# apache/tez

Measured on NVIDIA H100. Metric: sorted KV GB/s (16B key / 64B val), higher is better.
Workload: dtype u8

## Files before the change

### tez_b200/csrc/radix_sort.cuh

```cuda
#pragma once
#include "common.cuh"

#ifndef TEZGPU_RADIX_THREADS32
#define TEZGPU_RADIX_THREADS32 384
#endif
#ifndef TEZGPU_RADIX_IPT32
#define TEZGPU_RADIX_IPT32 16
#endif
#ifndef TEZGPU_RADIX_MINB32
#define TEZGPU_RADIX_MINB32 (1024 / TEZGPU_RADIX_THREADS32)
#endif
#ifndef TEZGPU_RADIX_LOOKBACK
#define TEZGPU_RADIX_LOOKBACK 4
#endif
#ifndef TEZGPU_RANK_MODE
#define TEZGPU_RANK_MODE 2
#endif

namespace tezgpu {

constexpr int RADIX_BITS = 8;
constexpr int RADIX = 1 << RADIX_BITS;
constexpr uint32_t STATE_FLAG_LOCAL = 1u << 30;
constexpr uint32_t STATE_FLAG_INCL = 2u << 30;
constexpr uint32_t STATE_VALUE_MASK = (1u << 30) - 1;
constexpr uint32_t RADIX_MAX_N = (1u << 30) - 1;

template <typename KeyT>
__device__ __forceinline__ uint32_t radix_digit(KeyT k, int shift) {
  return (uint32_t)(k >> shift) & (RADIX - 1);
}

template <typename KeyT, int NPASS>
__global__ void __launch_bounds__(512) k_radix_hist(const KeyT *__restrict__ keys, uint32_t n, int begin_bit,
                                                    uint32_t *__restrict__ hist ) {
  __shared__ uint32_t s_hist[NPASS * RADIX];
  for (int i = threadIdx.x; i < NPASS * RADIX; i += blockDim.x) s_hist[i] = 0;
  __syncthreads();
  uint32_t stride = gridDim.x * blockDim.x;
  for (uint32_t i = blockIdx.x * blockDim.x + threadIdx.x; i < n; i += stride) {
    KeyT k = keys[i];
#pragma unroll
    for (int p = 0; p < NPASS; p++) atomicAdd(&s_hist[p * RADIX + radix_digit(k, begin_bit + p * RADIX_BITS)], 1u);
  }
  __syncthreads();
  for (int i = threadIdx.x; i < NPASS * RADIX; i += blockDim.x) {
    uint32_t c = s_hist[i];
    if (c) atomicAdd(&hist[i], c);
  }
}

__global__ void __launch_bounds__(RADIX) k_radix_scan_hist(uint32_t *__restrict__ hist, int npass, uint32_t n,
                                                          uint32_t *__restrict__ trivial) {
  __shared__ uint32_t s_warp[RADIX / 32];
  const int tid = threadIdx.x, lane = tid & 31, warp = tid >> 5;
  for (int p = 0; p < npass; p++) {
    uint32_t c = hist[p * RADIX + tid];
    uint32_t incl = c;
#pragma unroll
    for (int o = 1; o < 32; o <<= 1) {
      uint32_t t = __shfl_up_sync(0xffffffffu, incl, o);
      if (lane >= o) incl += t;
    }
    if (lane == 31) s_warp[warp] = incl;
    __syncthreads();
    uint32_t base = 0;
    for (int w = 0; w < warp; w++) base += s_warp[w];
    hist[p * RADIX + tid] = base + incl - c;
    uint32_t any = __syncthreads_or(c == n && n > 0);
    if (tid == 0 && trivial) trivial[p] = any ? 1u : 0u;
    __syncthreads();
  }
}

enum RadixIO : int { IO_SEP = 0, IO_SEP_IOTA = 1, IO_PAIR = 2 };

template <typename KeyT, int THREADS, int IPT>
struct OnesweepCfg {
  static constexpr int NWARPS = THREADS / 32;
  static constexpr int TILE = THREADS * IPT;
  static constexpr size_t SMEM = (size_t)TILE * (sizeof(KeyT) + sizeof(uint32_t)) + (size_t)NWARPS * RADIX * 4 +
                                 2 * RADIX * 4 + 64 + (TEZGPU_RANK_MODE == 2 ? (size_t)NWARPS * RADIX * 4 : 0);
};

template <typename KeyT, int THREADS, int IPT, int MINB, int IN, int OUT>
__global__ void __launch_bounds__(THREADS, MINB)
    k_onesweep_pass(const KeyT *__restrict__ keys_in, KeyT *__restrict__ keys_out, const uint32_t *__restrict__ vals_in,
                    uint32_t *__restrict__ vals_out, uint32_t n, int shift, const uint32_t *__restrict__ hist_base,
                    uint32_t *tile_state, uint32_t *tile_counter) {
  using Cfg = OnesweepCfg<KeyT, THREADS, IPT>;
  constexpr int NWARPS = Cfg::NWARPS;
  constexpr int TILE = Cfg::TILE;
  constexpr bool PAIRS = sizeof(KeyT) == 4;
  static_assert(THREADS >= RADIX, "one thread per digit for the look-back");
  static_assert(PAIRS || (IN != IO_PAIR && OUT != IO_PAIR), "pairs carry 32-bit keys");
  static_assert(OUT != IO_SEP_IOTA, "iota is an input layout");

  extern __shared__ __align__(16) uint8_t smem_raw[];
  uint2 *s_pair = reinterpret_cast<uint2 *>(smem_raw);
  KeyT *s_keys = reinterpret_cast<KeyT *>(smem_raw);
  uint32_t *s_vals = reinterpret_cast<uint32_t *>(smem_raw + (size_t)TILE * sizeof(KeyT));
  uint32_t *s_wcnt = s_vals + TILE;
  uint32_t *s_dstart = s_wcnt + NWARPS * RADIX;
  uint32_t *s_goff = s_dstart + RADIX;
  uint32_t *s_misc = s_goff + RADIX;
#if TEZGPU_RANK_MODE == 2
  uint32_t *s_wmask = s_misc + 16;
#endif

  const int tid = threadIdx.x, lane = tid & 31, warp = tid >> 5;

#ifdef TEZGPU_TICKET_ATOMIC
  if (tid == 0) s_misc[0] = atomicAdd(tile_counter, 1u);
#else
  if (tid == 0) s_misc[0] = blockIdx.x;
#endif
  for (int i = tid; i < NWARPS * RADIX; i += THREADS) s_wcnt[i] = 0;
#if TEZGPU_RANK_MODE == 2
  for (int i = tid; i < NWARPS * RADIX; i += THREADS) s_wmask[i] = 0;
#endif
  __syncthreads();
  const uint32_t tile = s_misc[0];
  const uint32_t tile_base = tile * (uint32_t)TILE;
  const uint32_t tile_n = min((uint32_t)TILE, n - tile_base);
  const uint32_t warp_base = (uint32_t)warp * 32u * IPT;

  KeyT key[IPT];
  uint32_t val[IN == IO_SEP_IOTA ? 1 : IPT];
  uint32_t rnk[IPT];
#pragma unroll
  for (int j = 0; j < IPT; j++) {
    const uint32_t li = warp_base + j * 32 + lane;
    const bool valid = li < tile_n;
    if constexpr (IN == IO_PAIR) {
      uint2 p = make_uint2(~0u, 0u);
      if (valid) p = reinterpret_cast<const uint2 *>(keys_in)[tile_base + li];
      key[j] = p.x;
      val[j] = p.y;
    } else {
      key[j] = valid ? keys_in[tile_base + li] : ~(KeyT)0;
      if constexpr (IN == IO_SEP) val[j] = valid ? vals_in[tile_base + li] : 0u;
    }
  }
  uint32_t *wc = s_wcnt + warp * RADIX;
  const uint32_t lt = lanemask_lt();
#pragma unroll
  for (int j = 0; j < IPT; j++) {
    const uint32_t d = radix_digit(key[j], shift);
    uint32_t peers;
#if TEZGPU_RANK_MODE == 0
    peers = __match_any_sync(0xffffffffu, d);
#elif TEZGPU_RANK_MODE == 2
    {
      uint32_t *wm = s_wmask + warp * RADIX;
      atomicOr(&wm[d], 1u << lane);
      __syncwarp();
      peers = wm[d];
      __syncwarp();
      atomicAnd(&wm[d], ~(1u << lane));
    }
#else
    peers = 0xffffffffu;
#pragma unroll
    for (int b = 0; b < RADIX_BITS; b++) {
      const bool bit = (d >> b) & 1u;
      const uint32_t bm = __ballot_sync(0xffffffffu, bit);
      peers &= bit ? bm : ~bm;
    }
#endif
    uint32_t pre = 0;
    if ((peers & lt) == 0) pre = atomicAdd(&wc[d], (uint32_t)__popc(peers));
    pre = __shfl_sync(0xffffffffu, pre, __ffs(peers) - 1);
    rnk[j] = pre + __popc(peers & lt);
  }
  __syncthreads();

  uint32_t count = 0;
  if (tid < RADIX) {
    uint32_t run = 0;
#pragma unroll
    for (int w = 0; w < NWARPS; w++) {
      uint32_t c = s_wcnt[w * RADIX + tid];
      s_wcnt[w * RADIX + tid] = run;
      run += c;
    }
    count = run;
    st_relaxed_gpu_u32(&tile_state[(size_t)tile * RADIX + tid], (tile == 0 ? STATE_FLAG_INCL : STATE_FLAG_LOCAL) | count);
    uint32_t incl = count;
#pragma unroll
    for (int o = 1; o < 32; o <<= 1) {
      uint32_t t = __shfl_up_sync(0xffffffffu, incl, o);
      if (lane >= o) incl += t;
    }
    if (lane == 31) s_misc[1 + warp] = incl;
    s_dstart[tid] = incl - count;
  }
  __syncthreads();
  if (tid < RADIX) {
    uint32_t base = 0;
    for (int w = 0; w < warp; w++) base += s_misc[1 + w];
    s_dstart[tid] += base;
  }
  __syncthreads();

#pragma unroll
  for (int j = 0; j < IPT; j++) {
    const uint32_t d = radix_digit(key[j], shift);
    const uint32_t slot = s_dstart[d] + wc[d] + rnk[j];
    uint32_t v;
    if constexpr (IN == IO_SEP_IOTA) v = tile_base + warp_base + j * 32 + lane;
    else v = val[j];
    if constexpr (PAIRS) {
      s_pair[slot] = make_uint2((uint32_t)key[j], v);
    } else {
      s_keys[slot] = key[j];
      s_vals[slot] = v;
    }
  }

  if (tid < RADIX) {
    uint32_t excl = 0;
    if (tile > 0) {
      constexpr int LOOKBACK = TEZGPU_RADIX_LOOKBACK;
      int64_t t = (int64_t)tile - 1;
      bool done = false;
      while (!done) {
        uint32_t st[LOOKBACK];
#ifdef TEZGPU_RADIX_DEBUG
        if (tid == 0) atomicAdd(tile_counter + 7, 1u);
#endif
#pragma unroll
        for (int b = 0; b < LOOKBACK; b++)
          st[b] = (t - b >= 0) ? ld_relaxed_gpu_u32(&tile_state[(size_t)(t - b) * RADIX + tid]) : STATE_FLAG_INCL;
#pragma unroll
        for (int b = 0; b < LOOKBACK; b++) {
          if (done) break;
          uint32_t flag = st[b] & ~STATE_VALUE_MASK;
          if (flag == 0) break;
          excl += st[b] & STATE_VALUE_MASK;
          t--;
          if (flag == STATE_FLAG_INCL) done = true;
        }
      }
      st_relaxed_gpu_u32(&tile_state[(size_t)tile * RADIX + tid], STATE_FLAG_INCL | (excl + count));
    }
    s_goff[tid] = hist_base[tid] + excl - s_dstart[tid];
  }
  __syncthreads();

#pragma unroll
  for (int k = 0; k < IPT; k++) {
    const uint32_t slot = (uint32_t)tid + k * THREADS;
    if (slot < tile_n) {
      KeyT kk;
      uint32_t v;
      if constexpr (PAIRS) {
        const uint2 p = s_pair[slot];
        kk = p.x;
        v = p.y;
      } else {
        kk = s_keys[slot];
        v = s_vals[slot];
      }
      const uint32_t dest = s_goff[radix_digit(kk, shift)] + slot;
      if constexpr (OUT == IO_PAIR) {
        reinterpret_cast<uint2 *>(keys_out)[dest] = make_uint2((uint32_t)kk, v);
      } else {
        keys_out[dest] = kk;
        vals_out[dest] = v;
      }
    }
  }
}

struct RadixWorkspace {
  uint32_t *hist = nullptr;
  uint32_t *trivial = nullptr;
  uint32_t *tile_state = nullptr;
  uint32_t *tile_counter = nullptr;
  size_t tile_state_words = 0;
};

template <typename KeyT>
struct RadixTuning {
  static constexpr int THREADS = sizeof(KeyT) == 4 ? TEZGPU_RADIX_THREADS32 : 512;
  static constexpr int IPT = sizeof(KeyT) == 4 ? TEZGPU_RADIX_IPT32 : 10;
  static constexpr int MINB = sizeof(KeyT) == 4 ? TEZGPU_RADIX_MINB32 : 2;
};

template <typename KeyT>
static inline uint32_t radix_num_tiles(uint32_t n) {
  using T = RadixTuning<KeyT>;
  return (uint32_t)div_up(n, (uint64_t)T::THREADS * T::IPT);
}
template <typename KeyT>
static inline size_t radix_tile_state_words(uint32_t n, int npass) {
  return (size_t)radix_num_tiles<KeyT>(n) * RADIX * (size_t)npass;
}

template <typename KeyT, int IN, int OUT>
static void radix_launch_pass(cudaStream_t st, uint32_t ntiles, const KeyT *kin, KeyT *kout, const uint32_t *vin,
                              uint32_t *vout, uint32_t n, int shift, const uint32_t *hist, uint32_t *state,
                              uint32_t *counter) {
  using T = RadixTuning<KeyT>;
  using Cfg = OnesweepCfg<KeyT, T::THREADS, T::IPT>;
  auto kern = k_onesweep_pass<KeyT, T::THREADS, T::IPT, T::MINB, IN, OUT>;
  static bool attr_set = false;
  if (!attr_set) {
    TG_CUDA(cudaFuncSetAttribute(kern, cudaFuncAttributeMaxDynamicSharedMemorySize, (int)Cfg::SMEM));
    attr_set = true;
  }
  kern<<<ntiles, T::THREADS, Cfg::SMEM, st>>>(kin, kout, vin, vout, n, shift, hist, state, counter);
  TG_CUDA(cudaGetLastError());
}

template <typename KeyT>
static uint32_t radix_prepare(cudaStream_t st, const RadixWorkspace &ws, uint32_t n, int npass) {
  const uint32_t ntiles = radix_num_tiles<KeyT>(n);
  TG_CHECK((size_t)ntiles * RADIX * (size_t)npass <= ws.tile_state_words, -1, "radix workspace too small");
  TG_CUDA(cudaMemsetAsync(ws.tile_state, 0, (size_t)ntiles * RADIX * (size_t)npass * 4, st));
  TG_CUDA(cudaMemsetAsync(ws.tile_counter, 0, 8 * 4, st));
  return ntiles;
}


static int radix_sort_pairs(cudaStream_t st, const RadixWorkspace &ws, uint32_t *blk_a, uint32_t *blk_b, uint32_t n,
                            int begin_bit, int npass, uint32_t pass_mask, int *launches) {
  const int total = __builtin_popcount(pass_mask & ((1u << npass) - 1));
  TG_CHECK(total >= 1, -1, "radix sort without a pass");
  const uint32_t ntiles = radix_prepare<uint32_t>(st, ws, n, npass);
  int done = 0;
  for (int p = 0; p < npass; p++) {
    if (!((pass_mask >> p) & 1u)) continue;
    uint32_t *in = (done & 1) ? blk_b : blk_a, *out = (done & 1) ? blk_a : blk_b;
    const bool first = done == 0, last = done + 1 == total;
    const int shift = begin_bit + p * RADIX_BITS;
    const uint32_t *hist = ws.hist + p * RADIX;
    uint32_t *state = ws.tile_state + (size_t)p * ntiles * RADIX, *counter = ws.tile_counter + p;
    if (first && last)
      radix_launch_pass<uint32_t, IO_SEP_IOTA, IO_SEP>(st, ntiles, in, out, nullptr, out + n, n, shift, hist, state, counter);
    else if (first)
      radix_launch_pass<uint32_t, IO_SEP_IOTA, IO_PAIR>(st, ntiles, in, out, nullptr, nullptr, n, shift, hist, state, counter);
    else if (last)
      radix_launch_pass<uint32_t, IO_PAIR, IO_SEP>(st, ntiles, in, out, nullptr, out + n, n, shift, hist, state, counter);
    else
      radix_launch_pass<uint32_t, IO_PAIR, IO_PAIR>(st, ntiles, in, out, nullptr, nullptr, n, shift, hist, state, counter);
    if (launches) (*launches)++;
    done++;
  }
  return done;
}

template <typename KeyT>
static int radix_sort_passes(cudaStream_t st, const RadixWorkspace &ws, KeyT *keys_a, KeyT *keys_b, uint32_t *vals_a,
                             uint32_t *vals_b, uint32_t n, int begin_bit, int npass, uint32_t pass_mask, int *launches) {
  static_assert(sizeof(KeyT) == 8, "32-bit keys are sorted as pairs (radix_sort_pairs)");
  const uint32_t ntiles = radix_prepare<KeyT>(st, ws, n, npass);
  int done = 0;
  for (int p = 0; p < npass; p++) {
    if (!((pass_mask >> p) & 1u)) continue;
    KeyT *kin = (done & 1) ? keys_b : keys_a, *kout = (done & 1) ? keys_a : keys_b;
    uint32_t *vin = (done & 1) ? vals_b : vals_a, *vout = (done & 1) ? vals_a : vals_b;
    radix_launch_pass<KeyT, IO_SEP, IO_SEP>(st, ntiles, kin, kout, vin, vout, n, begin_bit + p * RADIX_BITS,
                                            ws.hist + p * RADIX, ws.tile_state + (size_t)p * ntiles * RADIX,
                                            ws.tile_counter + p);
    if (launches) (*launches)++;
    done++;
  }
  return done;
}

}
```

### tez_b200/csrc/scan.cuh

```cuda
#pragma once
#include "common.cuh"

namespace tezgpu {

constexpr int SCAN_THREADS = 256;
constexpr int SCAN_IPT = 8;
constexpr int SCAN_TILE = SCAN_THREADS * SCAN_IPT;

__device__ __forceinline__ uint64_t block_exclusive_scan_u64(uint64_t v, uint64_t *s_warp ,
                                                             uint64_t *total) {
  const int lane = threadIdx.x & 31, warp = threadIdx.x >> 5;
  uint64_t incl = v;
#pragma unroll
  for (int o = 1; o < 32; o <<= 1) {
    uint64_t t = __shfl_up_sync(0xffffffffu, incl, o);
    if (lane >= o) incl += t;
  }
  if (lane == 31) s_warp[warp] = incl;
  __syncthreads();
  uint64_t base = 0, tot = 0;
#pragma unroll
  for (int w = 0; w < SCAN_THREADS / 32; w++) {
    uint64_t x = s_warp[w];
    if (w < warp) base += x;
    tot += x;
  }
  __syncthreads();
  if (total) *total = tot;
  return base + incl - v;
}

__global__ void __launch_bounds__(1024) k_scan_block_sums(uint64_t *blk, uint32_t nblk) {
  __shared__ uint64_t s_warp[32];
  __shared__ uint64_t s_carry;
  const int lane = threadIdx.x & 31, warp = threadIdx.x >> 5;
  if (threadIdx.x == 0) s_carry = 0;
  __syncthreads();
  for (uint32_t base = 0; base < nblk; base += 1024) {
    uint32_t i = base + threadIdx.x;
    uint64_t v = i < nblk ? blk[i] : 0, incl = v;
#pragma unroll
    for (int o = 1; o < 32; o <<= 1) {
      uint64_t t = __shfl_up_sync(0xffffffffu, incl, o);
      if (lane >= o) incl += t;
    }
    if (lane == 31) s_warp[warp] = incl;
    __syncthreads();
    uint64_t wbase = 0, tot = 0;
    for (int w = 0; w < 32; w++) {
      uint64_t x = s_warp[w];
      if (w < warp) wbase += x;
      tot += x;
    }
    uint64_t carry = s_carry;
    if (i < nblk) blk[i] = carry + wbase + incl - v;
    __syncthreads();
    if (threadIdx.x == 0) s_carry = carry + tot;
    __syncthreads();
  }
  if (threadIdx.x == 0) blk[nblk] = s_carry;
}

__global__ void __launch_bounds__(SCAN_THREADS) k_sum_u32_blocks(const uint32_t *__restrict__ in, uint32_t n,
                                                                 uint64_t *__restrict__ blk) {
  __shared__ uint64_t s_warp[SCAN_THREADS / 32];
  uint32_t base = blockIdx.x * SCAN_TILE;
  uint64_t s = 0;
#pragma unroll
  for (int k = 0; k < SCAN_IPT; k++) {
    uint32_t i = base + k * SCAN_THREADS + threadIdx.x;
    if (i < n) s += in[i];
  }
  uint64_t tot;
  block_exclusive_scan_u64(s, s_warp, &tot);
  if (threadIdx.x == 0) blk[blockIdx.x] = tot;
}

__global__ void __launch_bounds__(SCAN_THREADS) k_scan_u32_apply(const uint32_t *__restrict__ in, uint32_t n,
                                                                 const uint64_t *__restrict__ blk,
                                                                 uint64_t *__restrict__ out) {
  __shared__ uint64_t s_warp[SCAN_THREADS / 32];
  uint32_t base = blockIdx.x * SCAN_TILE + threadIdx.x * SCAN_IPT;
  uint32_t v[SCAN_IPT];
  uint64_t s = 0;
#pragma unroll
  for (int k = 0; k < SCAN_IPT; k++) {
    uint32_t i = base + k;
    v[k] = i < n ? in[i] : 0;
    s += v[k];
  }
  uint64_t ex = block_exclusive_scan_u64(s, s_warp, nullptr) + blk[blockIdx.x];
#pragma unroll
  for (int k = 0; k < SCAN_IPT; k++) {
    uint32_t i = base + k;
    if (i < n) out[i] = ex;
    ex += v[k];
  }
  if (blockIdx.x == gridDim.x - 1 && threadIdx.x == SCAN_THREADS - 1) out[n] = blk[gridDim.x];
}

}
```

### tez_b200/csrc/sorter.cuh

```cuda
#pragma once
#include <stdlib.h>
#include <string.h>

#include <vector>

#include "../../include/tezgpu.h"
#include "device_util.h"
#include "combine.cuh"
#include "deflate.cuh"
#include "emit_pipe_u.cuh"
#include "sorter_kernels.cuh"

namespace tezgpu {

__global__ void k_store_to_host(uint32_t *__restrict__ dst0, const uint32_t *__restrict__ src0, uint32_t n0, uint32_t *__restrict__ dst1,
                                const uint32_t *__restrict__ src1, uint32_t n1, uint32_t *__restrict__ dst2,
                                const uint32_t *__restrict__ src2, uint32_t n2) {
  for (uint32_t i = threadIdx.x; i < n0; i += blockDim.x) dst0[i] = src0[i];
  for (uint32_t i = threadIdx.x; i < n1; i += blockDim.x) dst1[i] = src1[i];
  for (uint32_t i = threadIdx.x; i < n2; i += blockDim.x) dst2[i] = src2[i];
  __threadfence_system();
}
static inline void store_to_host(cudaStream_t st, void *d0, const void *s0, size_t b0, void *d1 = nullptr, const void *s1 = nullptr,
                                 size_t b1 = 0, void *d2 = nullptr, const void *s2 = nullptr, size_t b2 = 0) {
  k_store_to_host<<<1, 256, 0, st>>>((uint32_t *)d0, (const uint32_t *)s0, (uint32_t)(b0 / 4), (uint32_t *)d1, (const uint32_t *)s1,
                                     (uint32_t)(b1 / 4), (uint32_t *)d2, (const uint32_t *)s2, (uint32_t)(b2 / 4));
}


static inline int partition_bits(int P) {
  int b = 0;
  while ((1ll << b) < (long long)P) b++;
  return b;
}

struct DeviceConstants {
  CrcTables *d_crc = nullptr;
  static DeviceConstants &get(int device) {
    static DeviceConstants inst[64];
    DeviceConstants &d = inst[device & 63];
    if (!d.d_crc) {
      CrcTables *h = new CrcTables();
      crc_build_tables(*h, EMIT_CRC_STRIDE_WORDS);
      TG_CUDA(cudaMalloc((void **)&d.d_crc, sizeof(CrcTables)));
      TG_CUDA(cudaMemcpy(d.d_crc, h, sizeof(CrcTables), cudaMemcpyHostToDevice));
      delete h;
    }
    return d;
  }
};

struct FramingMismatch {};

enum class FixedEmitKernel {
  Pipe,
  Fast,
  PipeUnaligned,
  FastUnaligned,
  General,
};
struct FixedEmitPlan {
  FixedEmitKernel kernel;
  uint32_t recs_per_tile;
};

static inline FixedEmitPlan plan_fixed_emit(const Records &rec, uint32_t rec_size) {
  const uint32_t stride = rec.klen + rec.vlen, cpr = stride / 16;
  const uint32_t cap = std::max<uint32_t>(1, std::min<uint32_t>(EMIT_MAX_RECS, (FE_IMG_BYTES - 32) / rec_size));
  if (stride < 16 || stride % 16) return {FixedEmitKernel::General, cap};
  if (!rec.key_off && !rec.use_runs && ((uintptr_t)rec.kv & 15u) == 0) {
    const uint32_t m = emit4_max_recs(rec_size);
    if (emit4_fits(m, cpr, rec_size)) return {FixedEmitKernel::Pipe, std::min(cap, m)};
    return {FixedEmitKernel::Fast, cap};
  }
  const uint32_t m = emit4u_max_recs(cpr);
  if (m == 0) return {FixedEmitKernel::FastUnaligned, cap};
  const uint32_t top = std::min(cap, m);
  uint32_t best = top;
  double best_eff = 0;
  for (uint32_t r = top; r >= top - top / 10; r--) {
    const uint64_t chunks = ((uint64_t)r * rec_size + 15 + 4 + 2 + 15) / 16;
    const uint64_t rounds = (chunks + FE_THREADS - 1) / FE_THREADS;
    const double eff = (double)r / (double)rounds;
    if (eff > best_eff) { best_eff = eff; best = r; }
  }
  return {FixedEmitKernel::PipeUnaligned, best};
}

class SortPipeline {
 public:
  tezgpu_conf conf;
  int pbits;
  cudaStream_t stream = nullptr;
  EventTimer timer;
  int num_sms = 132;

  DeviceBuffer sortA, sortB, same, blk, small, tile_state, sizes, rec_off;
  DeviceBuffer t_pos[2], t_gid[2], t_lidx[2], t_key64[2], t_val[2], t_state, t_ghead, t_gneq, sym_sets, sym_tab, rep_flags;
  DeviceBuffer seg_start, tile_start, part_start, d_index, seg_crc, tile_desc, tile_crc, tie_state;
  PinnedBuffer h_small;

  explicit SortPipeline(const tezgpu_conf &c) : conf(c) {
    TG_CHECK(c.num_partitions >= 1, TEZGPU_E_INVALID, "num_partitions must be >= 1");
    TG_CHECK(c.comparator >= TEZGPU_CMP_BYTES && c.comparator <= TEZGPU_CMP_LONG, TEZGPU_E_UNSUPPORTED,
             "comparator outside the device-supported set (BYTES, TEXT, BYTESWRITABLE, INT, LONG)");
    TG_CHECK(c.partitioner == TEZGPU_PART_GIVEN || c.partitioner == TEZGPU_PART_HASH, TEZGPU_E_UNSUPPORTED,
             "partitioner outside the device-supported set (GIVEN, HASH)");
    int ndev = 0;
    cudaError_t e = cudaGetDeviceCount(&ndev);
    if (e != cudaSuccess || ndev == 0) {
      cudaGetLastError();
      throw Error(TEZGPU_E_CUDA, "no CUDA device available (libtezgpu has no CPU fallback)");
    }
    TG_CHECK(c.device >= 0 && c.device < ndev, TEZGPU_E_INVALID, "bad device ordinal");
    TG_CUDA(cudaSetDevice(c.device));
    TG_CUDA(cudaStreamCreateWithFlags(&stream, cudaStreamNonBlocking));
    TG_CUDA(cudaDeviceGetAttribute(&num_sms, cudaDevAttrMultiProcessorCount, c.device));
    {
      const char *g = getenv("TEZGPU_L2_FETCH");
      int gran = g ? atoi(g) : 32;
      if (gran > 0 && cudaDeviceSetLimit(cudaLimitMaxL2FetchGranularity, (size_t)gran) != cudaSuccess) cudaGetLastError();
    }
    pbits = partition_bits(c.num_partitions);
    TG_CHECK(pbits <= 31, TEZGPU_E_INVALID, "too many partitions");
    h_small.ensure(4096);
    small.ensure(16384);
    DeviceConstants::get(c.device);
  }
  ~SortPipeline() {
    if (stream) cudaStreamDestroy(stream);
  }

  static uint64_t output_bound(uint64_t n, uint64_t kv_bytes, int P) { return kv_bytes + 12 * n + 10ull * P + 64; }

  uint32_t *d_hist() { return small.as<uint32_t>(); }
  uint32_t *d_trivial() { return small.as<uint32_t>() + 2048; }
  uint32_t *d_tile_counter() { return small.as<uint32_t>() + 2056; }
  int *d_error() { return reinterpret_cast<int *>(small.as<uint32_t>() + 2064); }
  uint32_t *d_large() { return small.as<uint32_t>() + 2065; }
  uint32_t *d_m() { return small.as<uint32_t>() + 2072; }
  unsigned long long *d_ties() { return reinterpret_cast<unsigned long long *>(small.as<uint32_t>() + 2074); }
  uint32_t *d_ticket() { return small.as<uint32_t>() + 2073; }
  unsigned long long *d_dups() { return reinterpret_cast<unsigned long long *>(small.as<uint32_t>() + 2066); }
  uint64_t *d_totals() { return reinterpret_cast<uint64_t *>(small.as<uint32_t>() + 2068); }

  struct SortState {
    Records rec;
    uint32_t *K = nullptr;
    uint32_t *order = nullptr;
    uint64_t dup_count = 0, tie_records = 0;
    int launches = 0;
    bool have_bounds = false, spec_layout = false;
    uint64_t spec_file_bytes = 0, spec_tiles = 0;
    const uint8_t *same = nullptr;
  } state;
  int merge_check_same = 1;
  bool merge_inputs_plain = false;
  int combiner = TEZGPU_COMBINE_NONE;
  DeviceBuffer c_head, c_gid, c_sums, c_hpos, c_K, c_order, c_same, c_kv, c_koff, c_klen, c_vlen, c_bad;
  PinnedBuffer c_host;
  EventTimer c_timer;

  EmitParams make_emit_params(const Records &rec, const uint32_t *order, int rle, bool merge_mode, uint8_t *d_out) {
    EmitParams e;
    memset(&e, 0, sizeof(e));
    e.rec = rec;
    e.order = order;
    e.same = state.same ? state.same : same.as<uint8_t>();
    e.part_start = part_start.as<uint32_t>();
    e.seg_start = seg_start.as<uint64_t>();
    e.tile_start = tile_start.as<uint32_t>();
    e.out = d_out;
    e.seg_crc = seg_crc.as<uint32_t>();
    e.crc = DeviceConstants::get(conf.device).d_crc;
    e.rle = rle;
    e.send_empty = conf.send_empty_partition_details;
    e.unordered = conf.sorter_impl == TEZGPU_SORTER_UNORDERED;
    e.merge_mode = merge_mode ? 1 : 0;
    e.check_same = merge_check_same;
    e.P = conf.num_partitions;
    return e;
  }
  FixedEmitKernel set_fixed_layout(EmitParams &e, const Records &rec) {
    int h = 0;
    for (int b = 0; b < vint_size_u32(rec.klen); b++) e.fixed_hdr[h++] = vint_byte_u32(rec.klen, b);
    for (int b = 0; b < vint_size_u32(rec.vlen); b++) e.fixed_hdr[h++] = vint_byte_u32(rec.vlen, b);
    e.fixed_hdr_len = h;
    e.rec_size = h + rec.klen + rec.vlen;
    const FixedEmitPlan plan = plan_fixed_emit(rec, e.rec_size);
    e.recs_per_tile = plan.recs_per_tile;
    e.rec_off = nullptr;
    return plan.kernel;
  }

  void run(Records rec, uint8_t *d_out, uint64_t out_cap, uint64_t *out_len, int64_t *index, tezgpu_stats *stats) {
    const uint64_t raw_bound = output_bound(rec.n, rec.fixed ? (uint64_t)rec.n * (rec.klen + rec.vlen) : rec.kv_bytes, conf.num_partitions);
    sort_phase(rec);
    int rle;
    if (conf.rle_policy == TEZGPU_RLE_ON) rle = 1;
    else if (conf.rle_policy == TEZGPU_RLE_OFF) rle = 0;
    else rle = (conf.sorter_impl == 1) ? 0 : ((double)state.dup_count > 0.1 * (double)rec.n);
    if (conf.sorter_impl == TEZGPU_SORTER_UNORDERED) rle = 0;
    emit_out(rle, false, raw_bound, d_out, out_cap, out_len, index, stats);
  }

  int codec = TEZGPU_CODEC_NONE;
  DeviceBuffer z_img, z_slots, z_csize, z_cadler, z_coff, z_segs, z_descs, z_pstart, z_tc, z_crc;
  PinnedBuffer z_host;
  EventTimer z_timer;
  static uint64_t codec_bound(int codec, uint64_t raw_bound, int P);
  void compress_image(const int64_t *raw_index, uint8_t *d_out, uint64_t out_cap, uint64_t *out_len, int64_t *index, tezgpu_stats *stats);

  void emit_out(int rle, bool merge_mode, uint64_t raw_bound, uint8_t *d_out, uint64_t out_cap, uint64_t *out_len, int64_t *index,
                tezgpu_stats *stats) {
    if (!codec) {
      if (combiner) emit_combined(rle, d_out, out_cap, out_len, index, stats);
      else emit_phase(rle, merge_mode, d_out, out_cap, out_len, index, stats);
      return;
    }
    const int P = conf.num_partitions;
    z_img.ensure(raw_bound + 64);
    std::vector<int64_t> raw_index((size_t)P * 3, 0);
    uint64_t raw_len = 0;
    tezgpu_stats st;
    memset(&st, 0, sizeof(st));
    if (combiner) emit_combined(rle, z_img.as<uint8_t>(), z_img.cap, &raw_len, raw_index.data(), &st);
    else emit_phase(rle, merge_mode, z_img.as<uint8_t>(), z_img.cap, &raw_len, raw_index.data(), &st);
    compress_image(raw_index.data(), d_out, out_cap, out_len, index, &st);
    if (stats) *stats = st;
  }

  void sort_phase(Records rec) {
    TG_CUDA(cudaSetDevice(conf.device));
    const uint32_t n = rec.n;
    const int P = conf.num_partitions;
    TG_CHECK(n <= RADIX_MAX_N, TEZGPU_E_INVALID, "more than 2^30-1 records in one sort");
    rec.cmp = conf.comparator;
    rec.hash_partition = conf.partitioner == TEZGPU_PART_HASH;
    rec.num_partitions = P;
    rec.pbits = pbits;
    const bool unordered = conf.sorter_impl == TEZGPU_SORTER_UNORDERED;
    rec.unordered = unordered ? 1 : 0;
    TG_CHECK(rec.hash_partition || rec.partition || rec.use_runs || n == 0 || P == 1, TEZGPU_E_INVALID, "partition ids required (partitioner=GIVEN)");
    int launches = 0;
    state.have_bounds = state.spec_layout = false;
    state.same = nullptr;
    timer.reset();
    timer.mark(stream);

    const size_t n4 = (size_t)(n ? n : 1) * 4;
    sortA.ensure(2 * n4); sortB.ensure(2 * n4);
    same.ensure(n ? n : 1);
    const uint32_t nblk = (uint32_t)div_up(n ? n : 1, SCAN_TILE);
    blk.ensure(((size_t)nblk + 2) * 8);
    part_start.ensure(((size_t)P + 1) * 4);
    seg_start.ensure(((size_t)P + 1) * 8);
    tile_start.ensure(((size_t)P + 1) * 4);
    d_index.ensure((size_t)P * 24);
    seg_crc.ensure((size_t)P * 4);
    h_small.ensure(4096 + (size_t)P * 24);

    TG_CUDA(cudaMemsetAsync(small.p, 0, 16384, stream));
    TG_CUDA(cudaMemsetAsync(seg_crc.p, 0, (size_t)P * 4, stream));

    uint64_t dup_count = 0;
    uint64_t tie_records = 0;
    uint32_t *K = sortA.as<uint32_t>();
    uint32_t *order = sortA.as<uint32_t>() + n;

    uint32_t sym_npos = 0;
    if (n && !rec.fixed && !unordered && !(getenv("TEZGPU_NO_SYM") && atoi(getenv("TEZGPU_NO_SYM")))) {
      sym_sets.ensure(SYM_MAX_POS * 8 * 4);
      sym_tab.ensure(sizeof(SymTable));
      TG_CUDA(cudaMemsetAsync(sym_sets.p, 0, SYM_MAX_POS * 8 * 4, stream));
      k_symbols<<<(int)std::min<uint64_t>(div_up(n, 256), (uint64_t)num_sms * 8), 256, 0, stream>>>(rec, sym_sets.as<uint32_t>());
      launches++;
      uint32_t hs[SYM_MAX_POS * 8];
      TG_CUDA(cudaMemcpyAsync(hs, sym_sets.p, sizeof(hs), cudaMemcpyDeviceToHost, stream));
      TG_CUDA(cudaStreamSynchronize(stream));
      SymTable *t = new SymTable();
      const uint32_t np = sym_table_build(hs, pbits, t);
      if (sym_table_pays(np, pbits)) {
        TG_CUDA(cudaMemcpyAsync(sym_tab.p, t, sizeof(SymTable), cudaMemcpyHostToDevice, stream));
        TG_CUDA(cudaStreamSynchronize(stream));
        rec.sym = sym_tab.as<SymTable>();
        sym_npos = np;
      }
      delete t;
    }
    if (n) {
      TG_CUDA(cudaMemsetAsync(same.p, 0, n, stream));
      const bool fast16 = rec.fixed && !rec.key_off && !rec.use_runs && rec.klen == 16 && ((rec.klen + rec.vlen) % 16 == 0) && rec.cmp == CMP_BYTES &&
                          (((uintptr_t)rec.kv & 15u) == 0);
      int sgrid = (int)std::min<uint64_t>(div_up(n, 256), (uint64_t)num_sms * 16);
      if (fast16) k_stage<true><<<sgrid, 256, 0, stream>>>(rec, K, d_hist(), d_error());
      else k_stage<false><<<sgrid, 256, 0, stream>>>(rec, K, d_hist(), d_error());
      TG_CUDA(cudaGetLastError());
      k_radix_scan_hist<<<1, RADIX, 0, stream>>>(d_hist(), 4, n, d_trivial());
      TG_CUDA(cudaGetLastError());
      launches += 2;
      timer.mark(stream);

      RadixWorkspace ws;
      ws.hist = d_hist();
      ws.trivial = d_trivial();
      ws.tile_counter = d_tile_counter();
      ws.tile_state_words = radix_tile_state_words<uint32_t>(n, 4);
      tile_state.ensure(ws.tile_state_words * 4);
      ws.tile_state = tile_state.as<uint32_t>();
      uint32_t pass_mask = 0xF;
      if (unordered) {
        pass_mask = 0;
        for (int q = 0; q < 4; q++) if (8 * q + 8 > 32 - pbits) pass_mask |= 1u << q;
        if (!pass_mask) pass_mask = 1;
      }
      int done = radix_sort_pairs(stream, ws, sortA.as<uint32_t>(), sortB.as<uint32_t>(), n, 0, 4, pass_mask, &launches);
      if (done & 1) { K = sortB.as<uint32_t>(); order = sortB.as<uint32_t>() + n; }
      if (unordered) {
        k_flip_order<<<(uint32_t)div_up(n, 256), 256, 0, stream>>>(order, n);
        launches++;
      }
      timer.mark(stream);

      const uint32_t depth0 = rec.sym ? sym_npos : (uint32_t)((32 - pbits) / 8);
      int per_sm_tf = 0;
      TG_CUDA(cudaOccupancyMaxActiveBlocksPerMultiprocessor(&per_sm_tf, k_tie_fix, TIEFIX_THREADS, 0));
      if (!unordered)
        k_tie_fix<<<(uint32_t)std::min<uint64_t>(div_up(n, TIEFIX_TILE), (uint64_t)num_sms * std::max(per_sm_tf, 1)), TIEFIX_THREADS, 0, stream>>>(
            rec, K, order, n, depth0, same.as<uint8_t>(), d_dups(), d_large(), d_ties());
      const uint32_t *d_m_ptr = reinterpret_cast<const uint32_t *>(d_ties());
      k_part_bounds<<<(uint32_t)div_up((uint64_t)P + 1, 256), 256, 0, stream>>>(K, n, P, pbits, part_start.as<uint32_t>());
      launches += 2;
      state.have_bounds = true;
      state.spec_layout = false;
      if (rec.fixed) {
        EmitParams e = make_emit_params(rec, order, 0, false, nullptr);
        set_fixed_layout(e, rec);
        k_layout<<<1, 1024, 0, stream>>>(e, seg_start.as<uint64_t>(), tile_start.as<uint32_t>(), d_index.as<int64_t>(), d_totals());
        launches++;
        state.spec_layout = true;
      }
      TG_CUDA(cudaGetLastError());
      uint32_t *hw = h_small.as<uint32_t>();
      store_to_host(stream, hw, small.as<uint32_t>() + 2064, 32, hw + 8, d_m_ptr, 4, h_small.as<uint8_t>() + 4096, d_index.p,
                    state.spec_layout ? (size_t)P * 24 : 0);
      TG_CUDA(cudaGetLastError());
      TG_CUDA(cudaStreamSynchronize(stream));
      TG_CHECK(!(hw[0] & 1u), TEZGPU_E_INVALID, "Illegal partition (outside [0, numPartitions))");
      if (hw[0] & 2u) throw FramingMismatch();
      uint32_t m = hw[8];
      tie_records = m;
      memcpy(&dup_count, hw + 2, 8);
      memcpy(&state.spec_file_bytes, hw + 4, 8);
      memcpy(&state.spec_tiles, hw + 6, 8);
      uint64_t *hs = h_small.as<uint64_t>() + 16;
      if (hw[1]) {
        k_tie_count<<<nblk, SCAN_THREADS, 0, stream>>>(K, n, blk.as<uint64_t>());
        k_scan_block_sums<<<1, 1024, 0, stream>>>(blk.as<uint64_t>(), nblk);
        TG_CUDA(cudaMemcpyAsync(&hs[0], blk.as<uint64_t>() + nblk, 8, cudaMemcpyDeviceToHost, stream));
        TG_CUDA(cudaStreamSynchronize(stream));
        m = (uint32_t)hs[0];
        tie_records = m;
        for (int s2 = 0; s2 < 2; s2++) { t_pos[s2].ensure((size_t)m * 4); t_gid[s2].ensure((size_t)m * 4); t_lidx[s2].ensure((size_t)m * 4); }
        k_tie_compact<<<nblk, SCAN_THREADS, 0, stream>>>(K, order, n, blk.as<uint64_t>(), t_pos[0].as<uint32_t>(),
                                                         t_gid[0].as<uint32_t>(), t_lidx[0].as<uint32_t>());
        launches += 3;
        const uint32_t ngroups = (uint32_t)(hs[0] >> 32);
        int cur = 0;
        {
          t_ghead.ensure(((size_t)ngroups + 2) * 4);
          t_gneq.ensure((size_t)ngroups + 1);
          TG_CUDA(cudaMemsetAsync(t_gneq.p, 0, (size_t)ngroups + 1, stream));
          const uint32_t mgrid = (uint32_t)div_up(m, 256), mblk0 = (uint32_t)div_up(m, SCAN_TILE);
          k_group_heads<<<mgrid, 256, 0, stream>>>(t_gid[0].as<uint32_t>(), m, t_ghead.as<uint32_t>());
          k_group_equal<<<mgrid, 256, 0, stream>>>(rec, t_gid[0].as<uint32_t>(), t_lidx[0].as<uint32_t>(), t_ghead.as<uint32_t>(), m, depth0,
                                                 TIE_SMALL_MAX, t_gneq.as<uint8_t>());
          blk.ensure(((size_t)std::max(mblk0, nblk) + 2) * 8);
          k_group_mark<<<mblk0, SCAN_THREADS, 0, stream>>>(t_pos[0].as<uint32_t>(), t_gid[0].as<uint32_t>(), t_ghead.as<uint32_t>(),
                                                          t_gneq.as<uint8_t>(), m, TIE_SMALL_MAX, same.as<uint8_t>(), d_dups(), blk.as<uint64_t>());
          k_scan_block_sums<<<1, 1024, 0, stream>>>(blk.as<uint64_t>(), mblk0);
          launches += 4;
          TG_CUDA(cudaGetLastError());
          TG_CUDA(cudaMemcpyAsync(&hs[0], blk.as<uint64_t>() + mblk0, 8, cudaMemcpyDeviceToHost, stream));
          TG_CUDA(cudaStreamSynchronize(stream));
          const uint32_t m2 = (uint32_t)hs[0];
          if (m2) {
            k_group_compact<<<mblk0, SCAN_THREADS, 0, stream>>>(t_pos[0].as<uint32_t>(), t_gid[0].as<uint32_t>(), t_lidx[0].as<uint32_t>(),
                                                               t_ghead.as<uint32_t>(), t_gneq.as<uint8_t>(), m, TIE_SMALL_MAX, blk.as<uint64_t>(),
                                                               t_pos[1].as<uint32_t>(), t_gid[1].as<uint32_t>(), t_lidx[1].as<uint32_t>());
            launches++;
            TG_CUDA(cudaGetLastError());
            cur = 1;
          }
          m = m2;
        }
        uint32_t depth = depth0;
        while (m) {
          t_key64[0].ensure((size_t)m * 8); t_key64[1].ensure((size_t)m * 8); t_val[0].ensure((size_t)m * 4);
          const uint32_t mblk = (uint32_t)div_up(m, SCAN_TILE);
          k_ref_build_keys<<<(uint32_t)div_up(m, 256), 256, 0, stream>>>(rec, t_gid[cur].as<uint32_t>(), t_lidx[cur].as<uint32_t>(), m,
                                                                    depth, t_key64[0].as<uint64_t>());
          TG_CUDA(cudaMemsetAsync(d_hist(), 0, 8 * RADIX * 4, stream));
          k_radix_hist<uint64_t, 8><<<(int)std::min<uint64_t>(div_up(m, 512 * 8), (uint64_t)num_sms * 4), 512, 0, stream>>>(t_key64[0].as<uint64_t>(), m, 0, d_hist());
          k_radix_scan_hist<<<1, RADIX, 0, stream>>>(d_hist(), 8, m, d_trivial());
          launches += 3;
          TG_CUDA(cudaGetLastError());
          uint32_t *ht = h_small.as<uint32_t>() + 64;
          TG_CUDA(cudaMemcpyAsync(ht, d_trivial(), 8 * 4, cudaMemcpyDeviceToHost, stream));
          TG_CUDA(cudaStreamSynchronize(stream));
          uint32_t mask = 0;
          for (int q = 0; q < 8; q++) if (!ht[q]) mask |= 1u << q;
          RadixWorkspace w2 = ws;
          w2.tile_state_words = radix_tile_state_words<uint64_t>(m, 8);
          t_state.ensure(w2.tile_state_words * 4);
          w2.tile_state = t_state.as<uint32_t>();
          int d2 = radix_sort_passes<uint64_t>(stream, w2, t_key64[0].as<uint64_t>(), t_key64[1].as<uint64_t>(), t_lidx[cur].as<uint32_t>(),
                                               t_val[0].as<uint32_t>(), m, 0, 8, mask, &launches);
          const uint64_t *Ks = (d2 & 1) ? t_key64[1].as<uint64_t>() : t_key64[0].as<uint64_t>();
          const uint32_t *Ls = (d2 & 1) ? t_val[0].as<uint32_t>() : t_lidx[cur].as<uint32_t>();
          k_ref_apply_count<<<mblk, SCAN_THREADS, 0, stream>>>(Ks, Ls, t_pos[cur].as<uint32_t>(), m, order, same.as<uint8_t>(), d_dups(),
                                                              blk.as<uint64_t>());
          k_scan_block_sums<<<1, 1024, 0, stream>>>(blk.as<uint64_t>(), mblk);
          launches += 2;
          TG_CUDA(cudaMemcpyAsync(&hs[0], blk.as<uint64_t>() + mblk, 8, cudaMemcpyDeviceToHost, stream));
          TG_CUDA(cudaStreamSynchronize(stream));
          uint32_t m2 = (uint32_t)hs[0];
          if (m2) {
            k_ref_compact<<<mblk, SCAN_THREADS, 0, stream>>>(Ks, Ls, t_pos[cur].as<uint32_t>(), m, blk.as<uint64_t>(),
                                                            t_pos[cur ^ 1].as<uint32_t>(), t_gid[cur ^ 1].as<uint32_t>(),
                                                            t_lidx[cur ^ 1].as<uint32_t>());
            launches++;
            TG_CUDA(cudaGetLastError());
          }
          cur ^= 1;
          m = m2;
          depth += 3;
        }
        TG_CUDA(cudaMemcpyAsync(&hs[0], d_dups(), 8, cudaMemcpyDeviceToHost, stream));
        TG_CUDA(cudaStreamSynchronize(stream));
        dup_count = hs[0];
      }
    }
    timer.mark(stream);
    state.rec = rec;
    state.K = K;
    state.order = order;
    state.dup_count = dup_count;
    state.tie_records = tie_records;
    state.launches = launches;
  }

  void emit_phase(int rle, bool merge_mode, uint8_t *d_out, uint64_t out_cap, uint64_t *out_len, int64_t *index,
                  tezgpu_stats *stats) {
    TG_CUDA(cudaSetDevice(conf.device));
    TG_CHECK(((uintptr_t)d_out & 15u) == 0, TEZGPU_E_INVALID, "output buffer must be 16-byte aligned");
    const Records rec = state.rec;
    const uint32_t n = rec.n;
    const int P = conf.num_partitions;
    uint32_t *K = state.K, *order = state.order;
    const uint64_t dup_count = state.dup_count, tie_records = state.tie_records;
    int launches = state.launches;
    const CrcTables *d_crc = DeviceConstants::get(conf.device).d_crc;
    const size_t n4 = (size_t)(n ? n : 1) * 4;
    const uint32_t nblk = (uint32_t)div_up(n ? n : 1, SCAN_TILE);
    TG_CUDA(cudaMemsetAsync(seg_crc.p, 0, (size_t)P * 4, stream));
    if (timer.n > (n ? 4 : 2)) timer.n = n ? 4 : 2;

    EmitParams e = make_emit_params(rec, order, rle, merge_mode, d_out);
    if (!state.have_bounds) {
      k_part_bounds<<<(uint32_t)div_up((uint64_t)P + 1, 256), 256, 0, stream>>>(K, n, P, pbits, part_start.as<uint32_t>());
      launches++;
    }
    const bool no_repeats = !rle && (!merge_mode || (!merge_check_same && merge_inputs_plain));
    const bool fixed_emit = rec.fixed && (dup_count == 0 || no_repeats);
    uint64_t bound = output_bound(n, rec.fixed ? (uint64_t)n * (rec.klen + rec.vlen) : rec.kv_bytes, P);
    uint64_t *hs = h_small.as<uint64_t>();
    const FixedEmitKernel kernel = fixed_emit ? set_fixed_layout(e, rec) : FixedEmitKernel::General;
    if (fixed_emit && state.spec_layout) {
      hs[0] = state.spec_file_bytes;
      hs[1] = state.spec_tiles;
    } else {
      if (!fixed_emit) {
        uint64_t avg = n ? (rec.fixed ? (uint64_t)(rec.klen + rec.vlen) : rec.kv_bytes / n) + 4 : 16;
        e.recs_per_tile = (uint32_t)std::max<uint64_t>(1, std::min<uint64_t>(EMIT_MAX_RECS, (EMIT_IMG_BYTES - 32) / avg));
        sizes.ensure(n4);
        rec_off.ensure(((size_t)n + 2) * 8);
        if (n) {
          rep_flags.ensure(n);
          k_emit_repeat_flags<<<(uint32_t)div_up(n, 256), 256, 0, stream>>>(e, K, rep_flags.as<uint8_t>());
          launches++;
          e.rep = rep_flags.as<uint8_t>();
          k_emit_sizes<<<(uint32_t)div_up(n, 256), 256, 0, stream>>>(e, K, sizes.as<uint32_t>());
          k_sum_u32_blocks<<<nblk, SCAN_THREADS, 0, stream>>>(sizes.as<uint32_t>(), n, blk.as<uint64_t>());
          k_scan_block_sums<<<1, 1024, 0, stream>>>(blk.as<uint64_t>(), nblk);
          k_scan_u32_apply<<<nblk, SCAN_THREADS, 0, stream>>>(sizes.as<uint32_t>(), n, blk.as<uint64_t>(), rec_off.as<uint64_t>());
          launches += 4;
          TG_CUDA(cudaGetLastError());
        } else {
          TG_CUDA(cudaMemsetAsync(rec_off.p, 0, 16, stream));
        }
        e.rec_off = rec_off.as<uint64_t>();
      }
      k_layout<<<1, 1024, 0, stream>>>(e, seg_start.as<uint64_t>(), tile_start.as<uint32_t>(), d_index.as<int64_t>(), d_totals());
      launches++;
      TG_CUDA(cudaGetLastError());
      store_to_host(stream, &hs[0], d_totals(), 16, h_small.as<uint8_t>() + 4096, d_index.p, (size_t)P * 24);
      TG_CUDA(cudaGetLastError());
      TG_CUDA(cudaStreamSynchronize(stream));
      state.spec_layout = false;
    }
    const uint64_t file_bytes = hs[0];
    const uint64_t tiles = hs[1];
    TG_CHECK(file_bytes <= bound, TEZGPU_E_INVALID, "internal: output exceeds bound");
    TG_CHECK(file_bytes <= out_cap, TEZGPU_E_NOMEM, "output buffer too small for file.out");
    const bool source_oriented = fixed_emit && kernel != FixedEmitKernel::General;
    const uint32_t stride = rec.klen + rec.vlen;
    FastEmitParams fp;
    if (tiles && source_oriented) {
      tile_desc.ensure((size_t)tiles * sizeof(TileDesc));
      k_build_tiles<<<(uint32_t)div_up(tiles, 256), 256, 0, stream>>>(e, tile_desc.as<TileDesc>());
      launches++;
      fp.e = e;
      tile_crc.ensure((size_t)tiles * sizeof(TileCrc));
      fp.tile_crc = tile_crc.as<TileCrc>();
      fp.tiles = tile_desc.as<TileDesc>();
      fp.ntiles = (uint32_t)tiles;
      fp.cpr = stride / 16;
      fp.cpr_magic = fp.cpr == 1 ? 0u : (uint32_t)((1ull << 32) / fp.cpr) + 1u;
      fp.stride = stride;
    }
    timer.mark(stream);
    if (tiles) {
      auto persistent_grid = [&](auto kern, int threads, size_t smem) {
        int per_sm = 0;
        TG_CUDA(cudaOccupancyMaxActiveBlocksPerMultiprocessor(&per_sm, kern, threads, smem));
        return (uint32_t)std::min<uint64_t>(tiles, (uint64_t)num_sms * (per_sm > 0 ? per_sm : 1));
      };
      if (!fixed_emit) {
        k_emit<false><<<persistent_grid(k_emit<false>, EMIT_THREADS, 0), EMIT_THREADS, 0, stream>>>(e);
      } else {
        switch (kernel) {
          case FixedEmitKernel::Pipe: {
            static bool attr = false;
            if (!attr) {
              TG_CUDA(cudaFuncSetAttribute(k_emit_fast4<FE4_UNROLL>, cudaFuncAttributeMaxDynamicSharedMemorySize, (int)Emit4Smem::TOTAL));
              attr = true;
            }
            const uint32_t grid = (uint32_t)std::min<uint64_t>(div_up(tiles, FE4_GROUPS), (uint64_t)num_sms);
            k_emit_fast4<FE4_UNROLL><<<grid, FE_THREADS * FE4_GROUPS, Emit4Smem::TOTAL, stream>>>(fp);
            break;
          }
          case FixedEmitKernel::Fast:
            k_emit_fast<5, true><<<persistent_grid(k_emit_fast<5, true>, FE_THREADS, 0), FE_THREADS, 0, stream>>>(fp);
            break;
          case FixedEmitKernel::PipeUnaligned: {
            static bool attr = false;
            if (!attr) {
              TG_CUDA(cudaFuncSetAttribute(k_emit_fast4u<FE4U_UNROLL>, cudaFuncAttributeMaxDynamicSharedMemorySize, (int)Emit4uSmem::TOTAL));
              attr = true;
            }
            const uint32_t grid = persistent_grid(k_emit_fast4u<FE4U_UNROLL>, FE_THREADS, Emit4uSmem::TOTAL);
            k_emit_fast4u<FE4U_UNROLL><<<grid, FE_THREADS, Emit4uSmem::TOTAL, stream>>>(fp);
            break;
          }
          case FixedEmitKernel::FastUnaligned:
            k_emit_fast<5, false><<<persistent_grid(k_emit_fast<5, false>, FE_THREADS, 0), FE_THREADS, 0, stream>>>(fp);
            break;
          case FixedEmitKernel::General:
            k_emit<true><<<persistent_grid(k_emit<true>, EMIT_THREADS, 0), EMIT_THREADS, 0, stream>>>(e);
            break;
        }
      }
      if (source_oriented) {
        k_crc_combine<<<(uint32_t)div_up(tiles, 256), 256, 0, stream>>>(fp.tile_crc, (uint32_t)tiles, d_crc, seg_crc.as<uint32_t>());
        launches++;
      }
      launches++;
      TG_CUDA(cudaGetLastError());
    }
    timer.mark(stream);
    k_finalize_segments<<<(uint32_t)div_up(P, 256), 256, 0, stream>>>(e);
    launches++;
    TG_CUDA(cudaGetLastError());
    timer.mark(stream);
    TG_CUDA(cudaStreamSynchronize(stream));

    if (out_len) *out_len = file_bytes;
    const int64_t *hidx = reinterpret_cast<const int64_t *>(h_small.as<uint8_t>() + 4096);
    if (index) memcpy(index, hidx, (size_t)P * 24);
    if (stats) {
      memset(stats, 0, sizeof(*stats));
      stats->output_records = n;
      int64_t raw = 0;
      for (int p = 0; p < P; p++) raw += hidx[3 * p + 1];
      stats->output_bytes_with_overhead = raw;
      stats->output_bytes_physical = (int64_t)file_bytes;
      stats->file_out_bytes = (int64_t)file_bytes;
      stats->spilled_records = n;
      stats->num_spills = 1;
      stats->rle_used = rle;
      stats->adjacent_equal_keys = (int64_t)dup_count;
      stats->tie_records = (int64_t)tie_records;
      const int b = n ? 3 : 1;
      stats->ms_stage = n ? timer.ms(0, 1) : 0;
      stats->ms_sort = n ? timer.ms(1, 2) : 0;
      stats->ms_ties = n ? timer.ms(2, 3) : 0;
      stats->ms_emit = timer.ms(b, b + 3);
      stats->ms_emit_kernel = timer.ms(b + 1, b + 2);
      stats->ms_total = timer.ms(0, b + 3);
      stats->kernel_launches = launches;
    }
  }

  bool combine_phase() {
    const Records rec = state.rec;
    const uint32_t n = rec.n, W = combine_width(combiner);
    TG_CHECK(W, TEZGPU_E_INVALID, "unknown combiner");
    const char *name = combiner == TEZGPU_COMBINE_SUM_INT ? "IntSumReducer needs 4-byte IntWritable values"
                                                          : "LongSumReducer needs 8-byte LongWritable values";
    if (n == 0) return false;
    c_bad.ensure(16);
    c_host.ensure(64);
    uint32_t *bad = c_bad.as<uint32_t>();
    TG_CUDA(cudaMemsetAsync(bad, 0xFF, 4, stream));
    int launches = 0;
    if (state.dup_count == 0) {
      if (rec.fixed) {
        TG_CHECK(rec.vlen == W, TEZGPU_E_INVALID, "combiner: record 0 has a " + std::to_string(rec.vlen) + "-byte value (" + name + ")");
        return false;
      }
      k_combine_check_width<<<(uint32_t)std::min<uint64_t>(div_up(n, 256), (uint64_t)num_sms * 16), 256, 0, stream>>>(rec, W, bad);
      TG_CUDA(cudaGetLastError());
      state.launches += 1;
      uint32_t *h = c_host.as<uint32_t>();
      TG_CUDA(cudaMemcpyAsync(h, bad, 4, cudaMemcpyDeviceToHost, stream));
      TG_CUDA(cudaStreamSynchronize(stream));
      TG_CHECK(h[0] == 0xFFFFFFFFu, TEZGPU_E_INVALID, "combiner: record " + std::to_string(h[0]) + " has a value of the wrong width (" + name + ")");
      return false;
    }
    const uint32_t nblk = (uint32_t)div_up(n, SCAN_TILE);
    c_head.ensure((size_t)n * 4);
    c_gid.ensure(((size_t)n + 1) * 8);
    blk.ensure(((size_t)nblk + 2) * 8);
    k_combine_heads<<<(uint32_t)div_up(n, 256), 256, 0, stream>>>(same.as<uint8_t>(), n, c_head.as<uint32_t>());
    k_sum_u32_blocks<<<nblk, SCAN_THREADS, 0, stream>>>(c_head.as<uint32_t>(), n, blk.as<uint64_t>());
    k_scan_block_sums<<<1, 1024, 0, stream>>>(blk.as<uint64_t>(), nblk);
    k_scan_u32_apply<<<nblk, SCAN_THREADS, 0, stream>>>(c_head.as<uint32_t>(), n, blk.as<uint64_t>(), c_gid.as<uint64_t>());
    launches += 4;
    c_sums.ensure((size_t)n * 8);
    c_hpos.ensure((size_t)n * 4);
    c_K.ensure((size_t)n * 4);
    TG_CUDA(cudaMemsetAsync(c_sums.p, 0, (size_t)n * 8, stream));
    const uint32_t sgrid = (uint32_t)div_up(div_up(n, 32 * CMB_ROWS) * 32, CMB_THREADS);
    if (W == 4)
      k_combine_sum<4><<<sgrid, CMB_THREADS, 0, stream>>>(rec, state.order, state.K, c_gid.as<uint64_t>(), n, c_sums.as<unsigned long long>(),
                                                          c_hpos.as<uint32_t>(), c_K.as<uint32_t>(), bad);
    else
      k_combine_sum<8><<<sgrid, CMB_THREADS, 0, stream>>>(rec, state.order, state.K, c_gid.as<uint64_t>(), n, c_sums.as<unsigned long long>(),
                                                          c_hpos.as<uint32_t>(), c_K.as<uint32_t>(), bad);
    launches++;
    TG_CUDA(cudaGetLastError());
    uint32_t *h = c_host.as<uint32_t>();
    TG_CUDA(cudaMemcpyAsync(h, bad, 4, cudaMemcpyDeviceToHost, stream));
    TG_CUDA(cudaMemcpyAsync(h + 2, c_gid.as<uint64_t>() + n, 8, cudaMemcpyDeviceToHost, stream));
    TG_CUDA(cudaStreamSynchronize(stream));
    TG_CHECK(h[0] == 0xFFFFFFFFu, TEZGPU_E_INVALID, "combiner: record " + std::to_string(h[0]) + " has a value of the wrong width (" + name + ")");
    uint64_t m64;
    memcpy(&m64, h + 2, 8);
    const uint32_t m = (uint32_t)m64;
    c_order.ensure((size_t)m * 4);
    c_same.ensure(m);
    TG_CUDA(cudaMemsetAsync(c_same.p, 0, m, stream));
    Records out;
    memset(&out, 0, sizeof(out));
    out.n = m;
    out.cmp = rec.cmp;
    out.hash_partition = rec.hash_partition;
    out.num_partitions = rec.num_partitions;
    out.pbits = rec.pbits;
    const uint64_t *off = nullptr;
    uint64_t bytes;
    if (rec.fixed) {
      bytes = (uint64_t)m * (rec.klen + W);
      out.fixed = 1;
      out.klen = rec.klen;
      out.vlen = W;
    } else {
      const uint32_t mblk = (uint32_t)div_up(m, SCAN_TILE);
      k_combine_sizes<<<(uint32_t)div_up(m, 256), 256, 0, stream>>>(rec, state.order, c_hpos.as<uint32_t>(), m, W, c_head.as<uint32_t>());
      k_sum_u32_blocks<<<mblk, SCAN_THREADS, 0, stream>>>(c_head.as<uint32_t>(), m, blk.as<uint64_t>());
      k_scan_block_sums<<<1, 1024, 0, stream>>>(blk.as<uint64_t>(), mblk);
      k_scan_u32_apply<<<mblk, SCAN_THREADS, 0, stream>>>(c_head.as<uint32_t>(), m, blk.as<uint64_t>(), c_gid.as<uint64_t>());
      launches += 4;
      TG_CUDA(cudaGetLastError());
      TG_CUDA(cudaMemcpyAsync(h + 4, c_gid.as<uint64_t>() + m, 8, cudaMemcpyDeviceToHost, stream));
      TG_CUDA(cudaStreamSynchronize(stream));
      memcpy(&bytes, h + 4, 8);
      off = c_gid.as<uint64_t>();
      c_koff.ensure((size_t)m * 8);
      c_klen.ensure((size_t)m * 4);
      c_vlen.ensure((size_t)m * 4);
      out.key_off = c_koff.as<uint64_t>();
      out.key_len = c_klen.as<uint32_t>();
      out.val_len = c_vlen.as<uint32_t>();
    }
    c_kv.ensure(align_up(bytes, 16) + 32);
    out.kv = c_kv.as<uint8_t>();
    out.kv_bytes = rec.fixed ? bytes : align_up(bytes, 16);
    const bool narrow = rec.fixed && rec.klen <= 64;
    const uint32_t lanes = narrow ? 1 : 32;
    const uint32_t wgrid = (uint32_t)div_up((uint64_t)m * lanes, 256);
    auto write = [&](auto kern) {
      kern<<<wgrid, 256, 0, stream>>>(rec, state.order, c_hpos.as<uint32_t>(), c_sums.as<unsigned long long>(), m, off, c_kv.as<uint8_t>(),
                                      c_order.as<uint32_t>(), c_koff.as<uint64_t>(), c_klen.as<uint32_t>(), c_vlen.as<uint32_t>());
    };
    if (W == 4) narrow ? write(k_combine_write<4, 1>) : write(k_combine_write<4, 32>);
    else narrow ? write(k_combine_write<8, 1>) : write(k_combine_write<8, 32>);
    launches++;
    TG_CUDA(cudaGetLastError());
    state.rec = out;
    state.K = c_K.as<uint32_t>();
    state.order = c_order.as<uint32_t>();
    state.same = c_same.as<uint8_t>();
    state.dup_count = 0;
    state.have_bounds = state.spec_layout = false;
    state.launches += launches;
    return true;
  }

  void emit_combined(int rle, uint8_t *d_out, uint64_t out_cap, uint64_t *out_len, int64_t *index, tezgpu_stats *stats) {
    const SortState saved = state;
    c_timer.reset();
    c_timer.mark(stream);
    bool replaced = false;
    try {
      replaced = combine_phase();
      c_timer.mark(stream);
      emit_phase(rle, false, d_out, out_cap, out_len, index, stats);
    } catch (...) {
      restore_after_combine(saved, replaced);
      throw;
    }
    const uint64_t written = state.rec.n;
    restore_after_combine(saved, replaced);
    if (stats) {
      const float ms_combine = c_timer.ms(0, 1);
      stats->output_records = (int64_t)saved.rec.n;
      stats->spilled_records = (int64_t)written;
      stats->adjacent_equal_keys = (int64_t)saved.dup_count;
      stats->ms_emit = std::max(0.f, stats->ms_emit - ms_combine);
    }
  }
  void restore_after_combine(const SortState &saved, bool replaced) {
    if (!replaced) return;
    const int launches = state.launches;
    state = saved;
    state.launches = launches;
    state.have_bounds = state.spec_layout = false;
  }
};

}
```

### tez_b200/csrc/sorter_kernels.cuh

```cuda
#pragma once
#include "common.cuh"
#include "crc32.cuh"
#include "radix_sort.cuh"
#include "scan.cuh"

namespace tezgpu {

struct RunTable {
  const uint64_t *seg_off;
  const uint32_t *rec_base;
  const uint32_t *seg_part;
  const uint32_t *part_seg0;
  uint32_t nseg;
  uint32_t rec_size;
  uint32_t hdr_len;
  uint64_t hdr_bytes;
};

__device__ __forceinline__ uint32_t run_of(const RunTable &t, uint32_t i) {
  uint32_t lo = 0, hi = t.nseg;
  while (hi - lo > 1) {
    const uint32_t mid = (lo + hi) >> 1;
    if (__ldg(t.rec_base + mid) <= i) lo = mid; else hi = mid;
  }
  return lo;
}
__device__ __forceinline__ uint32_t run_of_in_partition(const RunTable &t, uint32_t p, uint32_t i) {
  uint32_t seg = __ldg(t.part_seg0 + p);
  const uint32_t end = __ldg(t.part_seg0 + p + 1);
  while (seg + 1 < end && i >= __ldg(t.rec_base + seg + 1)) seg++;
  return seg;
}
__device__ __forceinline__ uint64_t run_record_off(const RunTable &t, uint32_t i, uint32_t &seg) {
  seg = run_of(t, i);
  return __ldg(t.seg_off + seg) + (uint64_t)(i - __ldg(t.rec_base + seg)) * t.rec_size;
}
__device__ __forceinline__ uint64_t run_record_off_p(const RunTable &t, uint32_t p, uint32_t i) {
  const uint32_t seg = run_of_in_partition(t, p, i);
  return __ldg(t.seg_off + seg) + (uint64_t)(i - __ldg(t.rec_base + seg)) * t.rec_size;
}

constexpr int SYM_MAX_POS = 16;
struct SymTable {
  uint16_t rank[SYM_MAX_POS][256];
  uint8_t shift[SYM_MAX_POS];
  uint32_t npos;
};

static inline uint32_t sym_table_build(const uint32_t *sets, int pbits, SymTable *t) {
  memset(t, 0, sizeof(*t));
  const uint32_t avail = 32u - (uint32_t)pbits;
  uint32_t used = 0, np = 0;
  for (; np < (uint32_t)SYM_MAX_POS; np++) {
    uint32_t cnt = 0;
    for (int w = 0; w < 8; w++) cnt += (uint32_t)__builtin_popcount(sets[np * 8 + w]);
    if (cnt == 0) break;
    uint32_t bits = 0;
    while ((1u << bits) < cnt + 1) bits++;
    if (used + bits > avail) break;
    used += bits;
    t->shift[np] = (uint8_t)(avail - used);
    uint32_t rk = 0;
    for (uint32_t b = 0; b < 256; b++)
      if ((sets[np * 8 + (b >> 5)] >> (b & 31u)) & 1u) t->rank[np][b] = (uint16_t)(++rk);
  }
  t->npos = np;
  return np;
}
static inline bool sym_table_pays(uint32_t npos, int pbits) { return npos > (32u - (uint32_t)pbits) / 8u; }

struct Records {
  const uint8_t *kv;
  uint64_t kv_bytes;
  const uint64_t *key_off;
  const uint64_t *val_off;
  const uint32_t *key_len;
  const uint32_t *val_len;
  const int32_t *partition;
  const uint32_t *tag;
  uint32_t n;
  uint32_t klen, vlen;
  int fixed;
  int cmp;
  int hash_partition;
  int num_partitions;
  int pbits;
  int use_runs;
  RunTable runs;
  const SymTable *sym;
  int unordered;
};

__device__ __forceinline__ void record_lookup(const Records &r, uint32_t i, uint64_t &koff, uint32_t &klen,
                                              uint32_t &vlen) {
  if (r.fixed) {
    if (r.use_runs) {
      uint32_t seg;
      koff = run_record_off(r.runs, i, seg) + r.runs.hdr_len;
    } else {
      koff = r.key_off ? r.key_off[i] : (uint64_t)i * (r.klen + r.vlen);
    }
    klen = r.klen;
    vlen = r.vlen;
  } else {
    koff = r.key_off[i];
    klen = r.key_len[i];
    vlen = r.val_len[i];
  }
}

__device__ __forceinline__ uint32_t record_tag(const Records &r, uint32_t i) {
  return (r.fixed && r.use_runs) ? run_of(r.runs, i) << 1 : r.tag[i];
}

__host__ __device__ __forceinline__ uint32_t compose_sort_word(const Records &r, int32_t p, uint32_t prefix, bool &bad) {
  bad = p < 0 || p >= r.num_partitions;
  if (bad) p = 0;
  if (r.unordered) prefix = 0;
  return r.pbits ? (((uint32_t)p << (32 - r.pbits)) | (prefix >> r.pbits)) : prefix;
}

__host__ __device__ __forceinline__ uint32_t stage_sort_word(const Records &r, const uint8_t *key, uint32_t klen,
                                                             int32_t given, bool &bad) {
  const uint32_t skip = key_content_skip(r.cmp, key, klen);
  const uint8_t *content = key + skip;
  const uint32_t clen = klen - skip;
  uint32_t prefix = 0;
  if (r.sym) {
    const SymTable *__restrict__ st = r.sym;
    const uint32_t np = st->npos;
    for (uint32_t q = 0; q < np && q < clen; q++) prefix |= (uint32_t)st->rank[q][norm_byte(r.cmp, content, q)] << st->shift[q];
    prefix <<= r.pbits;
  } else {
#pragma unroll
    for (uint32_t b = 0; b < 4; b++) prefix = (prefix << 8) | (b < clen ? norm_byte(r.cmp, content, b) : 0u);
  }
  const int32_t p = r.hash_partition
                        ? (int32_t)((uint32_t)(key_hash_dev(r.cmp, key, klen) & 0x7fffffff) % (uint32_t)r.num_partitions)
                        : given;
  return compose_sort_word(r, p, prefix, bad);
}

template <bool FAST16>
__global__ void __launch_bounds__(256) k_stage(Records r, uint32_t *__restrict__ keys_out, uint32_t *__restrict__ hist,
                                               int *__restrict__ error_flag) {
  __shared__ uint32_t s_hist[4 * RADIX];
  for (int i = threadIdx.x; i < 4 * RADIX; i += blockDim.x) s_hist[i] = 0;
  __syncthreads();
  const uint32_t stride = gridDim.x * blockDim.x;
  for (uint32_t i = blockIdx.x * blockDim.x + threadIdx.x; i < r.n; i += stride) {
    uint32_t K;
    bool bad;
    if (FAST16) {
      const uint4 kq = *reinterpret_cast<const uint4 *>(r.kv + (uint64_t)i * (r.klen + r.vlen));
      const uint32_t prefix = __byte_perm(kq.x, 0, 0x0123);
      int32_t p;
      if (r.hash_partition) {
        uint32_t h = 1;
        const uint32_t w[4] = {kq.x, kq.y, kq.z, kq.w};
#pragma unroll
        for (int k = 0; k < 16; k++) h = 31u * h + (uint32_t)(int32_t)(int8_t)((w[k >> 2] >> (8 * (k & 3))) & 0xFF);
        p = (int32_t)((h & 0x7fffffffu) % (uint32_t)r.num_partitions);
      } else {
        p = r.partition ? r.partition[i] : 0;
      }
      K = compose_sort_word(r, p, prefix, bad);
    } else {
      uint64_t koff;
      uint32_t klen, vlen;
      int32_t run_part = 0;
      if (r.fixed && r.use_runs) {
        const unsigned am = __activemask();
        const int leader = __ffs(am) - 1;
        uint32_t seg = (int)(threadIdx.x & 31) == leader ? run_of(r.runs, i) : 0u;
        seg = __shfl_sync(am, seg, leader);
        while (seg + 1 < r.runs.nseg && i >= __ldg(r.runs.rec_base + seg + 1)) seg++;
        const uint64_t roff = __ldg(r.runs.seg_off + seg) + (uint64_t)(i - __ldg(r.runs.rec_base + seg)) * r.runs.rec_size;
        koff = roff + r.runs.hdr_len;
        klen = r.klen;
        vlen = r.vlen;
        run_part = (int32_t)__ldg(r.runs.seg_part + seg);
        bool ok = true;
        for (uint32_t b = 0; b < r.runs.hdr_len; b++) ok &= r.kv[roff + b] == (uint8_t)(r.runs.hdr_bytes >> (8 * b));
        if (!ok) atomicOr(error_flag, 2);
      } else {
        record_lookup(r, i, koff, klen, vlen);
      }
      const int32_t given = r.hash_partition ? 0 : ((r.fixed && r.use_runs) ? run_part : (r.partition ? r.partition[i] : 0));
      K = stage_sort_word(r, r.kv + koff, klen, given, bad);
    }
    if (bad) atomicOr(error_flag, 1);
    keys_out[r.unordered ? r.n - 1u - i : i] = K;
#pragma unroll
    for (int q = 0; q < 4; q++) atomicAdd(&s_hist[q * RADIX + ((K >> (8 * q)) & 0xFF)], 1u);
  }
  __syncthreads();
  for (int i = threadIdx.x; i < 4 * RADIX; i += blockDim.x) {
    uint32_t c = s_hist[i];
    if (c) atomicAdd(&hist[i], c);
  }
}

__global__ void __launch_bounds__(256) k_symbols(Records r, uint32_t *__restrict__ sets ) {
  __shared__ uint32_t s_set[SYM_MAX_POS * 8];
  for (int i = threadIdx.x; i < SYM_MAX_POS * 8; i += blockDim.x) s_set[i] = 0;
  __syncthreads();
  const uint32_t stride = gridDim.x * blockDim.x;
  for (uint32_t i = blockIdx.x * blockDim.x + threadIdx.x; i < r.n; i += stride) {
    uint64_t koff;
    uint32_t klen, vlen;
    record_lookup(r, i, koff, klen, vlen);
    const uint8_t *key = r.kv + koff;
    const uint32_t skip = key_content_skip(r.cmp, key, klen);
    const uint8_t *content = key + skip;
    const uint32_t clen = klen - skip;
    for (uint32_t q = 0; q < (uint32_t)SYM_MAX_POS && q < clen; q++) {
      const uint32_t b = norm_byte(r.cmp, content, q);
      const uint32_t bit = 1u << (b & 31u);
      if (!(s_set[q * 8 + (b >> 5)] & bit)) atomicOr(&s_set[q * 8 + (b >> 5)], bit);
    }
  }
  __syncthreads();
  for (int i = threadIdx.x; i < SYM_MAX_POS * 8; i += blockDim.x)
    if (s_set[i]) atomicOr(&sets[i], s_set[i]);
}

__device__ __forceinline__ void tie_flags(const uint32_t *__restrict__ K, uint32_t n, uint32_t i, bool &tied, bool &head) {
  uint32_t k = K[i];
  bool eq_prev = i > 0 && K[i - 1] == k;
  bool eq_next = i + 1 < n && K[i + 1] == k;
  tied = eq_prev || eq_next;
  head = tied && !eq_prev;
}

struct TileFlags {
  bool t[SCAN_IPT], h[SCAN_IPT];
};

__device__ __forceinline__ void tile_load_flags(const uint32_t *__restrict__ K, uint32_t n, uint32_t *s_k, TileFlags &f,
                                                uint32_t tile) {
  const uint32_t base = tile * SCAN_TILE;
  for (uint32_t i = threadIdx.x; i < SCAN_TILE + 2; i += SCAN_THREADS) {
    int64_t gi = (int64_t)base + i - 1;
    s_k[i] = (gi >= 0 && gi < (int64_t)n) ? K[gi] : 0u;
  }
  __syncthreads();
#pragma unroll
  for (int k = 0; k < SCAN_IPT; k++) {
    uint32_t li = k * SCAN_THREADS + threadIdx.x, i = base + li;
    f.t[k] = f.h[k] = false;
    if (i < n) {
      uint32_t v = s_k[li + 1];
      bool eq_prev = i > 0 && s_k[li] == v;
      bool eq_next = i + 1 < n && s_k[li + 2] == v;
      f.t[k] = eq_prev || eq_next;
      f.h[k] = f.t[k] && !eq_prev;
    }
  }
}

__global__ void __launch_bounds__(SCAN_THREADS) k_tie_count(const uint32_t *__restrict__ K, uint32_t n,
                                                            uint64_t *__restrict__ blk) {
  __shared__ uint32_t s_k[SCAN_TILE + 2];
  __shared__ uint64_t s_warp[SCAN_THREADS / 32];
  TileFlags f;
  tile_load_flags(K, n, s_k, f, blockIdx.x);
  uint64_t s = 0;
#pragma unroll
  for (int k = 0; k < SCAN_IPT; k++) s += (uint64_t)f.t[k] | ((uint64_t)f.h[k] << 32);
  uint64_t tot;
  block_exclusive_scan_u64(s, s_warp, &tot);
  if (threadIdx.x == 0) blk[blockIdx.x] = tot;
}

__global__ void __launch_bounds__(SCAN_THREADS)
    k_tie_compact(const uint32_t *__restrict__ K, const uint32_t *__restrict__ order, uint32_t n,
                  const uint64_t *__restrict__ blk, uint32_t *__restrict__ pos, uint32_t *__restrict__ gid,
                  uint32_t *__restrict__ lidx) {
  __shared__ uint32_t s_k[SCAN_TILE + 2];
  __shared__ uint32_t s_ct[SCAN_IPT][SCAN_THREADS / 32], s_ch[SCAN_IPT][SCAN_THREADS / 32];
  TileFlags f;
  tile_load_flags(K, n, s_k, f, blockIdx.x);
  const int lane = threadIdx.x & 31, warp = threadIdx.x >> 5;
  const uint32_t lt = lanemask_lt();
  uint32_t bt[SCAN_IPT], bh[SCAN_IPT];
#pragma unroll
  for (int k = 0; k < SCAN_IPT; k++) {
    bt[k] = __ballot_sync(0xffffffffu, f.t[k]);
    bh[k] = __ballot_sync(0xffffffffu, f.h[k]);
    if (lane == 0) { s_ct[k][warp] = __popc(bt[k]); s_ch[k][warp] = __popc(bh[k]); }
  }
  __syncthreads();
  const uint64_t b0 = blk[blockIdx.x];
  uint32_t run_t = (uint32_t)b0, run_h = (uint32_t)(b0 >> 32);
  const uint32_t base = blockIdx.x * SCAN_TILE;
#pragma unroll
  for (int k = 0; k < SCAN_IPT; k++) {
    uint32_t pre_t = run_t, pre_h = run_h;
#pragma unroll
    for (int w = 0; w < SCAN_THREADS / 32; w++) {
      uint32_t ct = s_ct[k][w], ch = s_ch[k][w];
      if (w < warp) { pre_t += ct; pre_h += ch; }
      run_t += ct; run_h += ch;
    }
    if (f.t[k]) {
      uint32_t at = pre_t + __popc(bt[k] & lt);
      uint32_t heads = pre_h + __popc(bh[k] & lt) + (f.h[k] ? 1u : 0u);
      uint32_t i = base + k * SCAN_THREADS + threadIdx.x;
      pos[at] = i;
      gid[at] = heads - 1;
      lidx[at] = order[i];
    }
  }
}

__global__ void __launch_bounds__(256) k_group_heads(const uint32_t *__restrict__ gid, uint32_t m, uint32_t *__restrict__ ghead) {
  const uint32_t j = blockIdx.x * blockDim.x + threadIdx.x;
  if (j >= m) return;
  const uint32_t g = gid[j];
  if (j == 0 || gid[j - 1] != g) ghead[g] = j;
  if (j + 1 == m) ghead[g + 1] = m;
}

__device__ __forceinline__ int compare_keys_from(const Records &r, uint32_t ra, uint32_t rb, uint32_t depth);

__global__ void __launch_bounds__(256)
    k_group_equal(Records r, const uint32_t *__restrict__ gid, const uint32_t *__restrict__ lidx, const uint32_t *__restrict__ ghead,
                  uint32_t m, uint32_t depth, uint32_t small_max, uint8_t *__restrict__ gneq) {
  const uint32_t j = blockIdx.x * blockDim.x + threadIdx.x;
  if (j >= m) return;
  const uint32_t g = gid[j], h = ghead[g];
  if (ghead[g + 1] - h <= small_max || j == h) return;
  if (compare_keys_from(r, lidx[h], lidx[j], depth) != 0) gneq[g] = 1;
}

__global__ void __launch_bounds__(SCAN_THREADS)
    k_group_mark(const uint32_t *__restrict__ pos, const uint32_t *__restrict__ gid, const uint32_t *__restrict__ ghead,
                 const uint8_t *__restrict__ gneq, uint32_t m, uint32_t small_max, uint8_t *__restrict__ same,
                 unsigned long long *__restrict__ dup_count, uint64_t *__restrict__ blk) {
  __shared__ uint64_t s_warp[SCAN_THREADS / 32];
  const uint32_t base = blockIdx.x * SCAN_TILE + threadIdx.x * SCAN_IPT;
  uint64_t sv = 0;
  uint32_t dups = 0;
#pragma unroll
  for (int k = 0; k < SCAN_IPT; k++) {
    const uint32_t j = base + k;
    if (j < m) {
      const uint32_t g = gid[j], h = ghead[g];
      if (ghead[g + 1] - h > small_max) {
        if (gneq[g]) sv += 1ull | ((uint64_t)(j == h) << 32);
        else if (j != h) { same[pos[j]] = 1; dups++; }
      }
    }
  }
  uint64_t tot;
  block_exclusive_scan_u64(sv, s_warp, &tot);
  if (threadIdx.x == 0) blk[blockIdx.x] = tot;
#pragma unroll
  for (int o = 16; o > 0; o >>= 1) dups += __shfl_xor_sync(0xffffffffu, dups, o);
  if ((threadIdx.x & 31) == 0 && dups) atomicAdd(dup_count, (unsigned long long)dups);
}

__global__ void __launch_bounds__(SCAN_THREADS)
    k_group_compact(const uint32_t *__restrict__ pos, const uint32_t *__restrict__ gid, const uint32_t *__restrict__ lidx,
                    const uint32_t *__restrict__ ghead, const uint8_t *__restrict__ gneq, uint32_t m, uint32_t small_max,
                    const uint64_t *__restrict__ blk, uint32_t *__restrict__ pos_out, uint32_t *__restrict__ gid_out,
                    uint32_t *__restrict__ lidx_out) {
  __shared__ uint64_t s_warp[SCAN_THREADS / 32];
  const uint32_t base = blockIdx.x * SCAN_TILE + threadIdx.x * SCAN_IPT;
  bool keep[SCAN_IPT], head[SCAN_IPT];
  uint64_t sv = 0;
#pragma unroll
  for (int k = 0; k < SCAN_IPT; k++) {
    const uint32_t j = base + k;
    keep[k] = head[k] = false;
    if (j < m) {
      const uint32_t g = gid[j], h = ghead[g];
      keep[k] = (ghead[g + 1] - h > small_max) && gneq[g];
      head[k] = keep[k] && j == h;
    }
    sv += (uint64_t)keep[k] | ((uint64_t)head[k] << 32);
  }
  const uint64_t ex = block_exclusive_scan_u64(sv, s_warp, nullptr) + blk[blockIdx.x];
  uint32_t at = (uint32_t)ex, heads = (uint32_t)(ex >> 32);
#pragma unroll
  for (int k = 0; k < SCAN_IPT; k++) {
    if (keep[k]) {
      if (head[k]) heads++;
      const uint32_t j = base + k;
      pos_out[at] = pos[j];
      gid_out[at] = heads - 1;
      lidx_out[at] = lidx[j];
      at++;
    }
  }
}

__device__ __forceinline__ int compare_keys_from(const Records &r, uint32_t ra, uint32_t rb, uint32_t depth) {
  uint64_t ka, kb;
  uint32_t la, lb, va, vb;
  record_lookup(r, ra, ka, la, va);
  record_lookup(r, rb, kb, lb, vb);
  const uint8_t *a = r.kv + ka, *b = r.kv + kb;
  uint32_t sa = key_content_skip(r.cmp, a, la), sb = key_content_skip(r.cmp, b, lb);
  a += sa; b += sb; la -= sa; lb -= sb;
  uint32_t nmin = la < lb ? la : lb;
  uint32_t i = depth;
  if (i == 0 && nmin > 0) {
    uint32_t x = norm_byte(r.cmp, a, 0), y = norm_byte(r.cmp, b, 0);
    if (x != y) return x < y ? -1 : 1;
    i = 1;
  }
  for (; i + 8 <= nmin; i += 8) {
    uint64_t x = 0, y = 0;
#pragma unroll
    for (int q = 0; q < 8; q++) {
      x = (x << 8) | a[i + q];
      y = (y << 8) | b[i + q];
    }
    if (x != y) return x < y ? -1 : 1;
  }
  for (; i < nmin; i++) {
    uint32_t x = a[i], y = b[i];
    if (x != y) return x < y ? -1 : 1;
  }
  return la < lb ? -1 : (la == lb ? 0 : 1);
}

constexpr uint32_t TIE_SMALL_MAX = 16;

constexpr int TIEFIX_THREADS = 256;
constexpr int TIEFIX_IPT = 8;
constexpr int TIEFIX_TILE = TIEFIX_THREADS * TIEFIX_IPT;

constexpr int TIEFIX_FLUSH = 4 * TIEFIX_THREADS;
constexpr int TIEFIX_CAP = TIEFIX_FLUSH + TIEFIX_TILE / 2 + 8;

__device__ __forceinline__ void tie_fix_group(const Records &r, const uint32_t *__restrict__ K, uint32_t *__restrict__ order,
                                              uint32_t n, uint32_t i, uint32_t depth, uint8_t *__restrict__ same,
                                              uint32_t &my_dups, uint32_t &my_ties, uint32_t *__restrict__ large_groups) {
  const uint32_t k = K[i];
  uint32_t e = i + 2;
  while (e < n && e - i <= TIE_SMALL_MAX && K[e] == k) e++;
  const uint32_t sz = e - i;
  if (sz > TIE_SMALL_MAX) { atomicAdd(large_groups, 1u); return; }
  my_ties += sz;
  uint32_t idx[TIE_SMALL_MAX];
  for (uint32_t j = 0; j < sz; j++) idx[j] = order[i + j];
  uint32_t eq = 0;
  for (uint32_t a = 1; a < sz; a++) {
    const uint32_t v = idx[a];
    uint32_t b = a;
    int c = 1;
    while (b > 0) {
      c = compare_keys_from(r, idx[b - 1], v, depth);
      if (c <= 0) break;
      idx[b] = idx[b - 1];
      b--;
    }
    idx[b] = v;
    const uint32_t low = eq & ((1u << b) - 1u);
    const uint32_t high = b < a ? ((eq >> (b + 1)) << (b + 2)) : 0u;
    eq = low | high | ((b > 0 && c == 0) ? (1u << b) : 0u);
  }
  order[i] = idx[0];
  for (uint32_t j = 1; j < sz; j++) {
    order[i + j] = idx[j];
    if ((eq >> j) & 1u) same[i + j] = 1;
  }
  my_dups += (uint32_t)__popc(eq);
}

__global__ void __launch_bounds__(TIEFIX_THREADS)
    k_tie_fix(Records r, const uint32_t *__restrict__ K, uint32_t *__restrict__ order, uint32_t n, uint32_t depth,
              uint8_t *__restrict__ same, unsigned long long *__restrict__ dup_count, uint32_t *__restrict__ large_groups,
              unsigned long long *__restrict__ tie_records) {
  __shared__ uint32_t s_heads[TIEFIX_CAP];
  __shared__ uint32_t s_nheads;
  const uint32_t ntiles = (n + TIEFIX_TILE - 1) / TIEFIX_TILE;
  if (threadIdx.x == 0) s_nheads = 0;
  __syncthreads();
  uint32_t my_dups = 0, my_ties = 0;
  for (uint32_t tile = blockIdx.x; tile < ntiles; tile += gridDim.x) {
    const uint32_t base = tile * TIEFIX_TILE;
    uint32_t kk[TIEFIX_IPT], kp[TIEFIX_IPT], kn[TIEFIX_IPT];
#pragma unroll
    for (int q = 0; q < TIEFIX_IPT; q++) {
      const uint32_t i = base + q * TIEFIX_THREADS + threadIdx.x;
      kk[q] = i < n ? __ldg(K + i) : 0u;
      kp[q] = (i > 0 && i < n) ? __ldg(K + i - 1) : ~kk[q];
      kn[q] = (i + 1 < n) ? __ldg(K + i + 1) : ~kk[q];
    }
#pragma unroll
    for (int q = 0; q < TIEFIX_IPT; q++) {
      const uint32_t i = base + q * TIEFIX_THREADS + threadIdx.x;
      if (i < n && kp[q] != kk[q] && kn[q] == kk[q]) s_heads[atomicAdd(&s_nheads, 1u)] = i;
    }
    __syncthreads();
    const uint32_t nh = s_nheads;
    const bool last = tile + gridDim.x >= ntiles;
    __syncthreads();
    if (nh >= (uint32_t)TIEFIX_FLUSH || last) {
      for (uint32_t hidx = threadIdx.x; hidx < nh; hidx += TIEFIX_THREADS)
        tie_fix_group(r, K, order, n, s_heads[hidx], depth, same, my_dups, my_ties, large_groups);
      __syncthreads();
      if (threadIdx.x == 0) s_nheads = 0;
      __syncthreads();
    }
  }
  if (my_dups) atomicAdd(dup_count, (unsigned long long)my_dups);
  if (my_ties) atomicAdd(tie_records, (unsigned long long)my_ties);
}

__device__ __forceinline__ uint32_t ref_subkey(const Records &r, uint32_t rec, uint32_t depth) {
  uint64_t koff;
  uint32_t klen, vlen;
  record_lookup(r, rec, koff, klen, vlen);
  const uint8_t *key = r.kv + koff;
  uint32_t skip = key_content_skip(r.cmp, key, klen);
  const uint8_t *content = key + skip;
  uint32_t clen = klen - skip;
  if (clen <= depth) return clen < 127u ? clen : 127u;
  uint32_t chunk = 0;
#pragma unroll
  for (uint32_t b = 0; b < 3; b++) chunk = (chunk << 8) | (depth + b < clen ? norm_byte(r.cmp, content, depth + b) : 0u);
  uint32_t rem = clen - depth;
  return (chunk << 8) | (128u + (rem < 3u ? rem : 3u));
}

__global__ void __launch_bounds__(256) k_ref_build_keys(Records r, const uint32_t *__restrict__ gid,
                                                        const uint32_t *__restrict__ lidx, uint32_t m, uint32_t depth,
                                                        uint64_t *__restrict__ key64) {
  uint32_t j = blockIdx.x * blockDim.x + threadIdx.x;
  if (j < m) key64[j] = ((uint64_t)gid[j] << 32) | ref_subkey(r, lidx[j], depth);
}

__device__ __forceinline__ void ref_flags(const uint64_t *__restrict__ K, uint32_t m, uint32_t j, bool &tied, bool &head,
                                          bool &open) {
  uint64_t k = K[j];
  bool eq_prev = j > 0 && K[j - 1] == k;
  bool eq_next = j + 1 < m && K[j + 1] == k;
  tied = eq_prev || eq_next;
  head = tied && !eq_prev;
  open = ((uint32_t)k & 0xFF) == 131u;
}

__global__ void __launch_bounds__(SCAN_THREADS)
    k_ref_apply_count(const uint64_t *__restrict__ K, const uint32_t *__restrict__ lidx_sorted,
                      const uint32_t *__restrict__ pos, uint32_t m, uint32_t *__restrict__ order,
                      uint8_t *__restrict__ same, unsigned long long *__restrict__ dup_count,
                      uint64_t *__restrict__ blk) {
  __shared__ uint64_t s_warp[SCAN_THREADS / 32];
  uint32_t base = blockIdx.x * SCAN_TILE + threadIdx.x * SCAN_IPT;
  uint64_t s = 0;
  uint32_t dups = 0;
#pragma unroll
  for (int k = 0; k < SCAN_IPT; k++) {
    uint32_t j = base + k;
    if (j < m) {
      bool t, h, open;
      ref_flags(K, m, j, t, h, open);
      uint32_t p = pos[j];
      order[p] = lidx_sorted[j];
      if (t && open) s += 1ull | ((uint64_t)h << 32);
      if (t && !open && !h) {
        same[p] = 1;
        dups++;
      }
    }
  }
  uint64_t tot;
  block_exclusive_scan_u64(s, s_warp, &tot);
  if (threadIdx.x == 0) blk[blockIdx.x] = tot;
#pragma unroll
  for (int o = 16; o > 0; o >>= 1) dups += __shfl_xor_sync(0xffffffffu, dups, o);
  if ((threadIdx.x & 31) == 0 && dups) atomicAdd(dup_count, (unsigned long long)dups);
}

__global__ void __launch_bounds__(SCAN_THREADS)
    k_ref_compact(const uint64_t *__restrict__ K, const uint32_t *__restrict__ lidx_sorted,
                  const uint32_t *__restrict__ pos, uint32_t m, const uint64_t *__restrict__ blk,
                  uint32_t *__restrict__ pos_out, uint32_t *__restrict__ gid_out, uint32_t *__restrict__ lidx_out) {
  __shared__ uint64_t s_warp[SCAN_THREADS / 32];
  uint32_t base = blockIdx.x * SCAN_TILE + threadIdx.x * SCAN_IPT;
  bool u[SCAN_IPT], h[SCAN_IPT];
  uint64_t s = 0;
#pragma unroll
  for (int k = 0; k < SCAN_IPT; k++) {
    uint32_t j = base + k;
    u[k] = h[k] = false;
    if (j < m) {
      bool t, hh, open;
      ref_flags(K, m, j, t, hh, open);
      u[k] = t && open;
      h[k] = u[k] && hh;
    }
    s += (uint64_t)u[k] | ((uint64_t)h[k] << 32);
  }
  uint64_t ex = block_exclusive_scan_u64(s, s_warp, nullptr) + blk[blockIdx.x];
  uint32_t at = (uint32_t)ex, heads = (uint32_t)(ex >> 32);
#pragma unroll
  for (int k = 0; k < SCAN_IPT; k++) {
    if (u[k]) {
      if (h[k]) heads++;
      uint32_t j = base + k;
      pos_out[at] = pos[j];
      gid_out[at] = heads - 1;
      lidx_out[at] = lidx_sorted[j];
      at++;
    }
  }
}

__global__ void k_flip_order(uint32_t *__restrict__ order, uint32_t n) {
  const uint32_t r = blockIdx.x * blockDim.x + threadIdx.x;
  if (r < n) order[r] = n - 1u - order[r];
}

__global__ void k_part_bounds(const uint32_t *__restrict__ K, uint32_t n, int P, int pbits,
                              uint32_t *__restrict__ part_start) {
  int p = blockIdx.x * blockDim.x + threadIdx.x;
  if (p > P) return;
  if (p == P) { part_start[p] = n; return; }
  if (pbits == 0) { part_start[p] = 0; return; }
  uint64_t target = (uint64_t)p << (32 - pbits);
  uint32_t lo = 0, hi = n;
  while (lo < hi) {
    uint32_t mid = lo + ((hi - lo) >> 1);
    if ((uint64_t)K[mid] < target) lo = mid + 1;
    else hi = mid;
  }
  part_start[p] = lo;
}

struct EmitParams {
  Records rec;
  const uint32_t *order;
  const uint8_t *same;
  const uint64_t *rec_off;
  const uint32_t *part_start;
  const uint64_t *seg_start;
  const uint32_t *tile_start;
  uint8_t *out;
  uint32_t *seg_crc;
  const CrcTables *crc;
  uint32_t recs_per_tile;
  uint32_t rec_size;
  uint8_t fixed_hdr[12];
  uint32_t fixed_hdr_len;
  int rle;
  int merge_mode;
  int check_same;
  int send_empty;
  int unordered;
  int P;
  const uint8_t *rep;
};

__device__ __forceinline__ bool emit_is_repeat(const EmitParams &e, uint32_t r, uint32_t ps) {
  if (e.rep) return e.rep[r] != 0;
  if (r == ps || !e.same[r]) return false;
  const Records &rec = e.rec;
  const uint32_t i = e.order[r];
  uint64_t koff;
  uint32_t klen, vlen;
  record_lookup(rec, i, koff, klen, vlen);
  const bool writer = e.rle && klen > 0;
  if (!e.merge_mode) return writer;
  const uint32_t tag = record_tag(rec, i);
  if (writer || (tag & 1u)) return true;
  return e.check_same && ((tag >> 1) != (record_tag(rec, e.order[r - 1]) >> 1));
}

__global__ void __launch_bounds__(256) k_emit_repeat_flags(EmitParams e, const uint32_t *__restrict__ K, uint8_t *__restrict__ flags) {
  const uint32_t r = blockIdx.x * blockDim.x + threadIdx.x;
  if (r >= e.rec.n) return;
  const int sh = 32 - e.rec.pbits;
  const uint32_t p = e.rec.pbits ? (K[r] >> sh) : 0;
  flags[r] = emit_is_repeat(e, r, e.part_start[p]) ? 1 : 0;
}

__global__ void __launch_bounds__(256) k_emit_sizes(EmitParams e, const uint32_t *__restrict__ K, uint32_t *__restrict__ sizes) {
  uint32_t r = blockIdx.x * blockDim.x + threadIdx.x;
  const Records &rec = e.rec;
  if (r >= rec.n) return;
  uint64_t koff;
  uint32_t klen, vlen;
  record_lookup(rec, e.order[r], koff, klen, vlen);
  const int sh = 32 - rec.pbits;
  const uint32_t p = rec.pbits ? (K[r] >> sh) : 0;
  const uint32_t ps = e.part_start[p], pe = e.part_start[p + 1];
  const bool last = (r + 1 == pe);
  const bool same_r = emit_is_repeat(e, r, ps);
  const bool same_prev = (r > ps) && emit_is_repeat(e, r - 1, ps);
  uint32_t sz;
  if (same_r) sz = (same_prev ? 0u : 1u) + vint_size_u32(vlen) + vlen;
  else sz = (same_prev ? 1u : 0u) + vint_size_u32(klen) + vint_size_u32(vlen) + klen + vlen;
  if (last && same_r) sz += 1;
  sizes[r] = sz;
}

__global__ void __launch_bounds__(1024)
    k_layout(EmitParams e, uint64_t *__restrict__ seg_start, uint32_t *__restrict__ tile_start,
             int64_t *__restrict__ index, uint64_t *__restrict__ totals ) {
  __shared__ uint64_t s_warp[32];
  __shared__ uint64_t s_carry_b;
  __shared__ uint64_t s_carry_t;
  const int lane = threadIdx.x & 31, warp = threadIdx.x >> 5;
  if (threadIdx.x == 0) { s_carry_b = 0; s_carry_t = 0; }
  __syncthreads();
  for (int base = 0; base < e.P; base += 1024) {
    int p = base + threadIdx.x;
    uint64_t seglen = 0, tiles = 0, body = 0;
    uint32_t cnt = 0;
    if (p < e.P) {
      uint32_t a = e.part_start[p], b = e.part_start[p + 1];
      cnt = b - a;
      if (cnt) {
        body = e.rec_off ? (e.rec_off[b] - e.rec_off[a]) : (uint64_t)cnt * e.rec_size;
        seglen = 4 + body + 2 + 4;
        tiles = (cnt + e.recs_per_tile - 1) / e.recs_per_tile;
      } else if (!e.send_empty && !e.unordered) {
        seglen = 10;
      }
    }
    uint64_t vb = seglen, ib = vb;
    uint64_t vt = tiles, it = vt;
#pragma unroll
    for (int o = 1; o < 32; o <<= 1) {
      uint64_t tb = __shfl_up_sync(0xffffffffu, ib, o);
      uint64_t tt = __shfl_up_sync(0xffffffffu, it, o);
      if (lane >= o) { ib += tb; it += tt; }
    }
    if (lane == 31) s_warp[warp] = ib;
    __syncthreads();
    uint64_t wb = 0, totb = 0;
    for (int w = 0; w < 32; w++) { uint64_t x = s_warp[w]; if (w < warp) wb += x; totb += x; }
    __syncthreads();
    if (lane == 31) s_warp[warp] = it;
    __syncthreads();
    uint64_t wt = 0, tott = 0;
    for (int w = 0; w < 32; w++) { uint64_t x = s_warp[w]; if (w < warp) wt += x; tott += x; }
    uint64_t cb = s_carry_b, ct = s_carry_t;
    if (p < e.P) {
      uint64_t start = cb + wb + ib - vb;
      seg_start[p] = start;
      tile_start[p] = (uint32_t)(ct + wt + it - vt);
      index[3 * p + 0] = (e.unordered && !seglen) ? 0 : (int64_t)start;
      index[3 * p + 1] = seglen ? (int64_t)(seglen - 4) : 0;
      index[3 * p + 2] = (int64_t)seglen;
    }
    __syncthreads();
    if (threadIdx.x == 0) { s_carry_b = cb + totb; s_carry_t = ct + tott; }
    __syncthreads();
  }
  if (threadIdx.x == 0) {
    seg_start[e.P] = s_carry_b;
    tile_start[e.P] = (uint32_t)s_carry_t;
    totals[0] = s_carry_b;
    totals[1] = s_carry_t;
  }
}

constexpr int EMIT_THREADS = 256;
constexpr int EMIT_MAX_RECS = 256;
constexpr int EMIT_IMG_BYTES = 24 * 1024;
constexpr int EMIT_CRC_STRIDE_WORDS = EMIT_THREADS;

struct EmitEntry {
  uint64_t src;
  uint64_t src2;
  uint32_t src_len;
  uint32_t src2_len;
  uint8_t hdr[12];
  uint8_t hdr_len;
  uint8_t tail_fd;
};

__device__ __forceinline__ uint4 load16_clamped(const uint8_t *p, const uint8_t *__restrict__ lo, const uint8_t *__restrict__ hi) {
  if (p >= lo && p + 16 <= hi) return *reinterpret_cast<const uint4 *>(p);
  uint32_t w[4] = {0, 0, 0, 0};
  for (int b = 0; b < 16; b++) {
    const uint8_t *q = p + b;
    if (q >= lo && q < hi) w[b >> 2] |= (uint32_t)(*q) << (8 * (b & 3));
  }
  return make_uint4(w[0], w[1], w[2], w[3]);
}

__device__ __forceinline__ void merge_bytes(uint32_t acc[4], const uint8_t *__restrict__ src, uint32_t o, uint32_t len,
                                            const uint8_t *__restrict__ lo, const uint8_t *__restrict__ hi) {
  const uint8_t *first = src - o;
  uint32_t sh = (uint32_t)((uintptr_t)first & 15u);
  const uint8_t *wb = first - sh;
  uint4 v0 = make_uint4(0, 0, 0, 0), v1 = make_uint4(0, 0, 0, 0);
  if (sh + o < 16u) v0 = load16_clamped(wb, lo, hi);
  if (sh + o + len > 16u) v1 = load16_clamped(wb + 16, lo, hi);
  const uint32_t bsh = (sh & 3u) * 8u;
  uint32_t r0, r1, r2, r3;
  switch (sh >> 2) {
    case 0:
      r0 = __funnelshift_r(v0.x, v0.y, bsh); r1 = __funnelshift_r(v0.y, v0.z, bsh);
      r2 = __funnelshift_r(v0.z, v0.w, bsh); r3 = __funnelshift_r(v0.w, v1.x, bsh);
      break;
    case 1:
      r0 = __funnelshift_r(v0.y, v0.z, bsh); r1 = __funnelshift_r(v0.z, v0.w, bsh);
      r2 = __funnelshift_r(v0.w, v1.x, bsh); r3 = __funnelshift_r(v1.x, v1.y, bsh);
      break;
    case 2:
      r0 = __funnelshift_r(v0.z, v0.w, bsh); r1 = __funnelshift_r(v0.w, v1.x, bsh);
      r2 = __funnelshift_r(v1.x, v1.y, bsh); r3 = __funnelshift_r(v1.y, v1.z, bsh);
      break;
    default:
      r0 = __funnelshift_r(v0.w, v1.x, bsh); r1 = __funnelshift_r(v1.x, v1.y, bsh);
      r2 = __funnelshift_r(v1.y, v1.z, bsh); r3 = __funnelshift_r(v1.z, v1.w, bsh);
      break;
  }
  const uint32_t rr[4] = {r0, r1, r2, r3};
  const uint32_t end = o + len;
#pragma unroll
  for (uint32_t w = 0; w < 4; w++) {
    uint32_t a = o > 4 * w ? o - 4 * w : 0u;
    uint32_t b = end < 4 * w + 4 ? (end > 4 * w ? end - 4 * w : 0u) : 4u;
    if (b > a) {
      uint32_t m = (0xFFFFFFFFu >> (8u * (4u - b))) & (0xFFFFFFFFu << (8u * a));
      acc[w] = (acc[w] & ~m) | (rr[w] & m);
    }
  }
}

__device__ __forceinline__ void put_byte(uint32_t acc[4], uint32_t q, uint32_t v) {
  uint32_t w = q >> 2, s = (q & 3u) * 8u;
#pragma unroll
  for (uint32_t k = 0; k < 4; k++)
    if (k == w) acc[k] = (acc[k] & ~(0xFFu << s)) | (v << s);
}

template <bool FIXED>
__global__ void __launch_bounds__(EMIT_THREADS) k_emit(EmitParams e) {
  __shared__ __align__(16) uint8_t s_img[EMIT_IMG_BYTES];
  __shared__ uint64_t s_loc[EMIT_MAX_RECS + 3];
  __shared__ EmitEntry s_ent[EMIT_MAX_RECS + 2];
  __shared__ uint32_t s_tab[4 * 256];
  __shared__ uint32_t s_adv[4 * 256];
  __shared__ uint32_t s_red[EMIT_THREADS / 32];
  __shared__ uint32_t s_info[8];

  const int tid = threadIdx.x;
  for (int i = tid; i < 4 * 256; i += EMIT_THREADS) {
    s_tab[i] = (&e.crc->slice[0][0])[i];
    s_adv[i] = (&e.crc->adv[0][0])[i];
  }
  const uint32_t ntiles = e.tile_start[e.P];
  for (uint32_t tile = blockIdx.x; tile < ntiles; tile += gridDim.x) {
  __syncthreads();

  if (tid == 0) {
    int lo = 0, hi = e.P;
    while (hi - lo > 1) {
      int mid = (lo + hi) >> 1;
      if (e.tile_start[mid] <= tile) lo = mid; else hi = mid;
    }
    while (lo + 1 < e.P && e.tile_start[lo + 1] <= tile) lo++;
    s_info[0] = (uint32_t)lo;
  }
  __syncthreads();
  const uint32_t p = s_info[0];
  const uint32_t ps = e.part_start[p], pe = e.part_start[p + 1];
  const uint32_t k = tile - e.tile_start[p];
  const uint32_t r0 = ps + k * e.recs_per_tile;
  const uint32_t nr = min(e.recs_per_tile, pe - r0);
  const bool first_tile = (k == 0), last_tile = (r0 + nr == pe);
  const Records &rec = e.rec;

  const uint64_t body0 = FIXED ? (uint64_t)(r0 - ps) * e.rec_size : (e.rec_off[r0] - e.rec_off[ps]);
  for (uint32_t j = tid; j < nr + 2; j += EMIT_THREADS) {
    EmitEntry en;
    en.src = 0; en.src_len = 0; en.src2 = 0; en.src2_len = 0; en.hdr_len = 0; en.tail_fd = 0;
    uint64_t loc;
    if (j == 0) {
      loc = 0;
      if (first_tile) { en.hdr[0] = 'T'; en.hdr[1] = 'I'; en.hdr[2] = 'F'; en.hdr[3] = 0; en.hdr_len = 4; }
    } else if (j == nr + 1) {
      uint64_t body_end = FIXED ? (uint64_t)(r0 - ps + nr) * e.rec_size : (e.rec_off[r0 + nr] - e.rec_off[ps]);
      loc = (first_tile ? 4 : 0) + (body_end - body0);
      if (last_tile) { en.hdr[0] = 0xFF; en.hdr[1] = 0xFF; en.hdr_len = 2; }
    } else {
      const uint32_t r = r0 + j - 1;
      uint64_t koff;
      uint32_t klen, vlen;
      record_lookup(rec, e.order[r], koff, klen, vlen);
      if (FIXED) {
        loc = (first_tile ? 4 : 0) + (uint64_t)(j - 1) * e.rec_size;
        for (uint32_t b = 0; b < e.fixed_hdr_len; b++) en.hdr[b] = e.fixed_hdr[b];
        en.hdr_len = (uint8_t)e.fixed_hdr_len;
        en.src = koff;
        en.src_len = klen + vlen;
      } else {
        loc = (first_tile ? 4 : 0) + (e.rec_off[r] - e.rec_off[ps]) - body0;
        const bool last = (r + 1 == pe);
        const bool same_r = emit_is_repeat(e, r, ps);
        const bool same_prev = (r > ps) && emit_is_repeat(e, r - 1, ps);
        uint32_t h = 0;
        if (same_r) {
          if (!same_prev) en.hdr[h++] = 0xFE;
          int s = vint_size_u32(vlen);
          for (int b = 0; b < s; b++) en.hdr[h++] = vint_byte_u32(vlen, b);
          en.src = (rec.val_off && !rec.fixed) ? rec.val_off[e.order[r]] : koff + klen;
          en.src_len = vlen;
          en.tail_fd = last ? 1 : 0;
        } else {
          if (same_prev) en.hdr[h++] = 0xFD;
          int s = vint_size_u32(klen);
          for (int b = 0; b < s; b++) en.hdr[h++] = vint_byte_u32(klen, b);
          s = vint_size_u32(vlen);
          for (int b = 0; b < s; b++) en.hdr[h++] = vint_byte_u32(vlen, b);
          en.src = koff;
          if (rec.val_off && !rec.fixed) { en.src_len = klen; en.src2 = rec.val_off[e.order[r]]; en.src2_len = vlen; }
          else en.src_len = klen + vlen;
        }
        en.hdr_len = (uint8_t)h;
      }
    }
    s_ent[j] = en;
    s_loc[j] = loc;
    if (j == nr + 1) s_loc[nr + 2] = loc + en.hdr_len;
  }
  __syncthreads();

  const uint32_t nent = nr + 2;
  const uint64_t tile_bytes = s_loc[nent];
  const uint64_t abs0 = e.seg_start[p] + (first_tile ? 0 : 4 + body0);
  const uint64_t seg_body_end = e.seg_start[p + 1] - 4;
  const uint8_t *kv_lo = rec.kv, *kv_hi = rec.kv + rec.kv_bytes;

  uint64_t done = 0;
  while (done < tile_bytes) {
    const uint64_t abs_piece = abs0 + done;
    const uint32_t lead = (uint32_t)(abs_piece & 15u);
    const uint32_t plen = (uint32_t)min((uint64_t)(EMIT_IMG_BYTES - lead), tile_bytes - done);
    const uint32_t nchunks = (lead + plen + 15u) >> 4;

    for (uint32_t c = tid; c < nchunks; c += EMIT_THREADS) {
      uint32_t acc[4] = {0, 0, 0, 0};
      uint64_t x0 = done + (c == 0 ? 0u : 16u * c - lead);
      const uint64_t x1 = min(done + (uint64_t)plen, done + (uint64_t)(16u * (c + 1) - lead));
      uint32_t q = (c == 0) ? lead : 0u;
      uint32_t j;
      if (FIXED) {
        uint64_t hdr = first_tile ? 4 : 0;
        j = x0 < hdr ? 0u : (uint32_t)min((uint64_t)nr, (x0 - hdr) / e.rec_size) + 1u;
        while (j + 1 < nent && s_loc[j + 1] <= x0) j++;
      } else {
        uint32_t lo = 0, hi = nent;
        while (hi - lo > 1) {
          uint32_t mid = (lo + hi) >> 1;
          if (s_loc[mid] <= x0) lo = mid; else hi = mid;
        }
        j = lo;
      }
      while (x0 < x1 && j < nent) {
        const uint64_t e_end = s_loc[j + 1];
        if (e_end <= x0) { j++; continue; }
        const uint64_t stop = min(x1, e_end);
        const EmitEntry &en = s_ent[j];
        uint32_t y = (uint32_t)(x0 - s_loc[j]);
        uint32_t left = (uint32_t)(stop - x0);
        while (left && y < en.hdr_len) { put_byte(acc, q, en.hdr[y]); y++; q++; left--; }
        if (left && y < en.hdr_len + en.src_len) {
          uint32_t take = min(left, en.hdr_len + en.src_len - y);
          merge_bytes(acc, kv_lo + en.src + (y - en.hdr_len), q, take, kv_lo, kv_hi);
          y += take; q += take; left -= take;
        }
        if (left && y < en.hdr_len + en.src_len + en.src2_len) {
          uint32_t take = min(left, en.hdr_len + en.src_len + en.src2_len - y);
          merge_bytes(acc, kv_lo + en.src2 + (y - en.hdr_len - en.src_len), q, take, kv_lo, kv_hi);
          y += take; q += take; left -= take;
        }
        if (left) { put_byte(acc, q, 0xFDu); q++; left--; }
        x0 = stop;
        j++;
      }
      *reinterpret_cast<uint4 *>(s_img + 16u * c) = make_uint4(acc[0], acc[1], acc[2], acc[3]);
    }
    __syncthreads();

    uint32_t cb0 = lead, cb1 = lead + plen;
    if (first_tile && done < 4) cb0 = min(cb1, lead + (uint32_t)(4 - done));
    {
      const uint32_t wa = (cb0 + 3u) >> 2, wb = cb1 >> 2;
      uint32_t c_thread = 0;
      uint32_t c_head = 0, n_tailbytes = 0;
      const uint32_t *img32 = reinterpret_cast<const uint32_t *>(s_img);
      if (wb > wa) {
        const uint32_t W = wb - wa;
        if ((uint32_t)tid < W) {
          uint32_t i = wa + tid;
          uint32_t c = 0;
          for (; i + EMIT_CRC_STRIDE_WORDS < wb; i += EMIT_CRC_STRIDE_WORDS) {
            uint32_t v = c ^ img32[i];
            c = s_adv[v & 0xFF] ^ s_adv[256 + ((v >> 8) & 0xFF)] ^ s_adv[512 + ((v >> 16) & 0xFF)] ^ s_adv[768 + (v >> 24)];
          }
          uint32_t v = c ^ img32[i];
          c = s_tab[768 + (v & 0xFF)] ^ s_tab[512 + ((v >> 8) & 0xFF)] ^ s_tab[256 + ((v >> 16) & 0xFF)] ^ s_tab[v >> 24];
          uint32_t d = wb - 1 - i;
          if (d) c = crc_multmodp(c, e.crc->pow_word[d]);
          c_thread = c;
        }
        if (tid == 0) {
          n_tailbytes = cb1 - 4 * wb;
        }
      }
#pragma unroll
      for (int o = 16; o > 0; o >>= 1) c_thread ^= __shfl_xor_sync(0xffffffffu, c_thread, o);
      if ((tid & 31) == 0) s_red[tid >> 5] = c_thread;
      __syncthreads();
      if (tid == 0) {
        uint32_t words_crc = 0;
        for (int w = 0; w < EMIT_THREADS / 32; w++) words_crc ^= s_red[w];
        uint32_t raw = 0;
        uint32_t head_end = (wb > wa) ? 4 * wa : cb1;
        for (uint32_t b = cb0; b < head_end; b++) raw = s_tab[(raw ^ s_img[b]) & 0xFF] ^ (raw >> 8);
        if (wb > wa) {
          raw = crc_shift_bytes(e.crc, raw, 4ull * (wb - wa)) ^ words_crc;
          for (uint32_t b = 4 * wb; b < cb1; b++) raw = s_tab[(raw ^ s_img[b]) & 0xFF] ^ (raw >> 8);
        }
        (void)c_head; (void)n_tailbytes;
        const uint32_t nbody = cb1 - cb0;
        if (nbody) {
          const uint64_t after = seg_body_end - (abs_piece + plen);
          uint32_t contrib = crc_shift_bytes(e.crc, raw, after);
          atomicXor(&e.seg_crc[p], contrib);
        }
      }
    }

    uint8_t *dst = e.out + (abs_piece - lead);
    for (uint32_t c = tid; c < nchunks; c += EMIT_THREADS) {
      uint32_t b0 = 16u * c, b1 = b0 + 16u;
      if (b0 >= lead && b1 <= lead + plen) {
        *reinterpret_cast<uint4 *>(dst + b0) = *reinterpret_cast<const uint4 *>(s_img + b0);
      } else {
        uint32_t a = max(b0, lead), b = min(b1, lead + plen);
        for (uint32_t x = a; x < b; x++) dst[x] = s_img[x];
      }
    }
    __syncthreads();
    done += plen;
  }
  }
}

__global__ void k_finalize_segments(EmitParams e) {
  int p = blockIdx.x * blockDim.x + threadIdx.x;
  if (p >= e.P) return;
  uint64_t s0 = e.seg_start[p], s1 = e.seg_start[p + 1];
  if (s1 == s0) return;
  uint32_t cnt = e.part_start[p + 1] - e.part_start[p];
  uint8_t *o = e.out + s0;
  uint32_t crc;
  if (cnt == 0) {
    o[0] = 'T'; o[1] = 'I'; o[2] = 'F'; o[3] = 0; o[4] = 0xFF; o[5] = 0xFF;
    crc = 0xFFFF0000u;
    o += 6;
  } else {
    uint64_t body = s1 - s0 - 8;
    crc = e.seg_crc[p] ^ crc_shift_bytes(e.crc, 0xFFFFFFFFu, body) ^ 0xFFFFFFFFu;
    o += s1 - s0 - 4;
  }
  o[0] = (uint8_t)(crc >> 24); o[1] = (uint8_t)(crc >> 16); o[2] = (uint8_t)(crc >> 8); o[3] = (uint8_t)crc;
}

}
```

Measured before the change: 501.8.

## Fuse first radix pass into staging kernel via tile-local sort and run descriptors

The staging kernel now sorts each tile locally by the first digit and writes (key, index) pairs tile-sorted, plus per-digit per-tile counts and starts. Separate kernels then build run descriptors, so the next onesweep pass reads pairs by gathering runs (IO_RUNS) rather than doing a full scatter pass for that digit. The aim is to remove one global scatter pass and its memory traffic. In exchange it adds extra count and build kernels, more shared-memory and register use in staging, and more complex indexing that could go wrong.

After: 516.0 (median of 6 runs). 1.03x the previous value.

```diff
diff --git a/tez_b200/csrc/radix_sort.cuh b/tez_b200/csrc/radix_sort.cuh
--- a/tez_b200/csrc/radix_sort.cuh
+++ b/tez_b200/csrc/radix_sort.cuh
@@ -1,5 +1,8 @@
 #pragma once
+#include <utility>
+
 #include "common.cuh"
+#include "scan.cuh"
 
 #ifndef TEZGPU_RADIX_THREADS32
 #define TEZGPU_RADIX_THREADS32 384
@@ -73,7 +76,12 @@
   }
 }
 
-enum RadixIO : int { IO_SEP = 0, IO_SEP_IOTA = 1, IO_PAIR = 2 };
+enum RadixIO : int { IO_SEP = 0, IO_RUNS = 1, IO_PAIR = 2 };
+
+struct RadixRuns {
+  const uint2 *desc = nullptr;
+  const uint32_t *first = nullptr;
+};
 
 template <typename KeyT, int THREADS, int IPT>
 struct OnesweepCfg {
@@ -83,66 +91,37 @@
                                  2 * RADIX * 4 + 64 + (TEZGPU_RANK_MODE == 2 ? (size_t)NWARPS * RADIX * 4 : 0);
 };
 
-template <typename KeyT, int THREADS, int IPT, int MINB, int IN, int OUT>
-__global__ void __launch_bounds__(THREADS, MINB)
-    k_onesweep_pass(const KeyT *__restrict__ keys_in, KeyT *__restrict__ keys_out, const uint32_t *__restrict__ vals_in,
-                    uint32_t *__restrict__ vals_out, uint32_t n, int shift, const uint32_t *__restrict__ hist_base,
-                    uint32_t *tile_state, uint32_t *tile_counter) {
+template <typename KeyT, int THREADS, int IPT>
+struct TileSmem {
   using Cfg = OnesweepCfg<KeyT, THREADS, IPT>;
-  constexpr int NWARPS = Cfg::NWARPS;
-  constexpr int TILE = Cfg::TILE;
+  uint2 *pair;
+  KeyT *keys;
+  uint32_t *vals;
+  uint32_t *wcnt;
+  uint32_t *dstart;
+  uint32_t *goff;
+  uint32_t *misc;
+  uint32_t *wmask;
+  __device__ __forceinline__ explicit TileSmem(uint8_t *raw) {
+    pair = reinterpret_cast<uint2 *>(raw);
+    keys = reinterpret_cast<KeyT *>(raw);
+    vals = reinterpret_cast<uint32_t *>(raw + (size_t)Cfg::TILE * sizeof(KeyT));
+    wcnt = vals + Cfg::TILE;
+    dstart = wcnt + Cfg::NWARPS * RADIX;
+    goff = dstart + RADIX;
+    misc = goff + RADIX;
+    wmask = misc + 16;
+  }
+};
+
+template <typename KeyT, int THREADS, int IPT, typename ValOf, typename Publish>
+__device__ __forceinline__ uint32_t tile_rank_reorder(const TileSmem<KeyT, THREADS, IPT> &s, const KeyT (&key)[IPT],
+                                                      int shift, ValOf val_of, Publish publish) {
+  constexpr int NWARPS = THREADS / 32;
   constexpr bool PAIRS = sizeof(KeyT) == 4;
-  static_assert(THREADS >= RADIX, "one thread per digit for the look-back");
-  static_assert(PAIRS || (IN != IO_PAIR && OUT != IO_PAIR), "pairs carry 32-bit keys");
-  static_assert(OUT != IO_SEP_IOTA, "iota is an input layout");
-
-  extern __shared__ __align__(16) uint8_t smem_raw[];
-  uint2 *s_pair = reinterpret_cast<uint2 *>(smem_raw);
-  KeyT *s_keys = reinterpret_cast<KeyT *>(smem_raw);
-  uint32_t *s_vals = reinterpret_cast<uint32_t *>(smem_raw + (size_t)TILE * sizeof(KeyT));
-  uint32_t *s_wcnt = s_vals + TILE;
-  uint32_t *s_dstart = s_wcnt + NWARPS * RADIX;
-  uint32_t *s_goff = s_dstart + RADIX;
-  uint32_t *s_misc = s_goff + RADIX;
-#if TEZGPU_RANK_MODE == 2
-  uint32_t *s_wmask = s_misc + 16;
-#endif
-
   const int tid = threadIdx.x, lane = tid & 31, warp = tid >> 5;
-
-#ifdef TEZGPU_TICKET_ATOMIC
-  if (tid == 0) s_misc[0] = atomicAdd(tile_counter, 1u);
-#else
-  if (tid == 0) s_misc[0] = blockIdx.x;
-#endif
-  for (int i = tid; i < NWARPS * RADIX; i += THREADS) s_wcnt[i] = 0;
-#if TEZGPU_RANK_MODE == 2
-  for (int i = tid; i < NWARPS * RADIX; i += THREADS) s_wmask[i] = 0;
-#endif
-  __syncthreads();
-  const uint32_t tile = s_misc[0];
-  const uint32_t tile_base = tile * (uint32_t)TILE;
-  const uint32_t tile_n = min((uint32_t)TILE, n - tile_base);
-  const uint32_t warp_base = (uint32_t)warp * 32u * IPT;
-
-  KeyT key[IPT];
-  uint32_t val[IN == IO_SEP_IOTA ? 1 : IPT];
   uint32_t rnk[IPT];
-#pragma unroll
-  for (int j = 0; j < IPT; j++) {
-    const uint32_t li = warp_base + j * 32 + lane;
-    const bool valid = li < tile_n;
-    if constexpr (IN == IO_PAIR) {
-      uint2 p = make_uint2(~0u, 0u);
-      if (valid) p = reinterpret_cast<const uint2 *>(keys_in)[tile_base + li];
-      key[j] = p.x;
-      val[j] = p.y;
-    } else {
-      key[j] = valid ? keys_in[tile_base + li] : ~(KeyT)0;
-      if constexpr (IN == IO_SEP) val[j] = valid ? vals_in[tile_base + li] : 0u;
-    }
-  }
-  uint32_t *wc = s_wcnt + warp * RADIX;
+  uint32_t *wc = s.wcnt + warp * RADIX;
   const uint32_t lt = lanemask_lt();
 #pragma unroll
   for (int j = 0; j < IPT; j++) {
@@ -152,7 +131,7 @@
     peers = __match_any_sync(0xffffffffu, d);
 #elif TEZGPU_RANK_MODE == 2
     {
-      uint32_t *wm = s_wmask + warp * RADIX;
+      uint32_t *wm = s.wmask + warp * RADIX;
       atomicOr(&wm[d], 1u << lane);
       __syncwarp();
       peers = wm[d];
@@ -180,43 +159,151 @@
     uint32_t run = 0;
 #pragma unroll
     for (int w = 0; w < NWARPS; w++) {
-      uint32_t c = s_wcnt[w * RADIX + tid];
-      s_wcnt[w * RADIX + tid] = run;
+      uint32_t c = s.wcnt[w * RADIX + tid];
+      s.wcnt[w * RADIX + tid] = run;
       run += c;
     }
     count = run;
-    st_relaxed_gpu_u32(&tile_state[(size_t)tile * RADIX + tid], (tile == 0 ? STATE_FLAG_INCL : STATE_FLAG_LOCAL) | count);
+    publish(count);
     uint32_t incl = count;
 #pragma unroll
     for (int o = 1; o < 32; o <<= 1) {
       uint32_t t = __shfl_up_sync(0xffffffffu, incl, o);
       if (lane >= o) incl += t;
     }
-    if (lane == 31) s_misc[1 + warp] = incl;
-    s_dstart[tid] = incl - count;
+    if (lane == 31) s.misc[1 + warp] = incl;
+    s.dstart[tid] = incl - count;
   }
   __syncthreads();
   if (tid < RADIX) {
     uint32_t base = 0;
-    for (int w = 0; w < warp; w++) base += s_misc[1 + w];
-    s_dstart[tid] += base;
+    for (int w = 0; w < warp; w++) base += s.misc[1 + w];
+    s.dstart[tid] += base;
   }
   __syncthreads();
 
 #pragma unroll
   for (int j = 0; j < IPT; j++) {
     const uint32_t d = radix_digit(key[j], shift);
-    const uint32_t slot = s_dstart[d] + wc[d] + rnk[j];
-    uint32_t v;
-    if constexpr (IN == IO_SEP_IOTA) v = tile_base + warp_base + j * 32 + lane;
-    else v = val[j];
+    const uint32_t slot = s.dstart[d] + wc[d] + rnk[j];
     if constexpr (PAIRS) {
-      s_pair[slot] = make_uint2((uint32_t)key[j], v);
+      s.pair[slot] = make_uint2((uint32_t)key[j], val_of(j));
     } else {
-      s_keys[slot] = key[j];
-      s_vals[slot] = v;
-    }
-  }
+      s.keys[slot] = key[j];
+      s.vals[slot] = val_of(j);
+    }
+  }
+  return count;
+}
+
+template <int THREADS, int IPT>
+__device__ __forceinline__ void load_run_items(const uint2 *__restrict__ blk, const RadixRuns &runs, uint32_t tile,
+                                               uint32_t tile_base, uint32_t tile_n, uint2 *s_runs, uint32_t *s_bits,
+                                               uint2 (&item)[IPT]) {
+  constexpr uint32_t TILE = (uint32_t)THREADS * IPT;
+  static_assert(IPT <= 32, "one lane per row of a warp");
+  const uint32_t k0 = __ldg(runs.first + tile);
+  const uint32_t cnt = min(__ldg(runs.first + tile + 1) - k0 + 1u, TILE);
+  for (uint32_t i = threadIdx.x; i < cnt; i += THREADS) {
+    const uint2 r = __ldg(runs.desc + k0 + i);
+    s_runs[i] = r;
+    const uint32_t l = r.x - tile_base;
+    if (l < TILE) atomicOr(&s_bits[l >> 5], 1u << (l & 31u));
+  }
+  __syncthreads();
+  const uint32_t lane = threadIdx.x & 31u, row0 = (threadIdx.x >> 5) * IPT;
+  uint32_t before = 0;
+  for (uint32_t w = lane; w < row0; w += 32) before += __popc(s_bits[w]);
+  before = __reduce_add_sync(0xffffffffu, before);
+  const uint32_t mybits = lane < (uint32_t)IPT ? s_bits[row0 + lane] : 0u;
+  uint32_t incl = __popc(mybits);
+#pragma unroll
+  for (int o = 1; o < 32; o <<= 1) {
+    const uint32_t t = __shfl_up_sync(0xffffffffu, incl, o);
+    if (lane >= (uint32_t)o) incl += t;
+  }
+  const uint32_t mypre = before + incl - __popc(mybits) - (s_runs[0].x == tile_base ? 1u : 0u);
+  const uint32_t le = lanemask_lt() | (1u << lane);
+  const uint32_t pos0 = tile_base + row0 * 32u + lane;
+#pragma unroll
+  for (int j = 0; j < IPT; j++) {
+    const uint32_t bits = __shfl_sync(0xffffffffu, mybits, j), pre = __shfl_sync(0xffffffffu, mypre, j);
+    const uint32_t pos = pos0 + j * 32u;
+    item[j] = make_uint2(~0u, 0u);
+    if (pos - tile_base < tile_n) {
+      const uint2 r = s_runs[pre + __popc(bits & le)];
+      item[j] = blk[r.y + (pos - r.x)];
+    }
+  }
+}
+
+template <typename KeyT, int THREADS, int IPT, int MINB, int IN, int OUT>
+__global__ void __launch_bounds__(THREADS, MINB)
+    k_onesweep_pass(const KeyT *__restrict__ keys_in, KeyT *__restrict__ keys_out, const uint32_t *__restrict__ vals_in,
+                    uint32_t *__restrict__ vals_out, uint32_t n, int shift, const uint32_t *__restrict__ hist_base,
+                    uint32_t *tile_state, uint32_t *tile_counter, RadixRuns runs) {
+  using Cfg = OnesweepCfg<KeyT, THREADS, IPT>;
+  constexpr int NWARPS = Cfg::NWARPS;
+  constexpr int TILE = Cfg::TILE;
+  constexpr bool PAIRS = sizeof(KeyT) == 4;
+  static_assert(THREADS >= RADIX, "one thread per digit for the look-back");
+  static_assert(PAIRS || (IN == IO_SEP && OUT == IO_SEP), "pairs and runs carry 32-bit keys");
+  static_assert(OUT != IO_RUNS, "runs are an input layout");
+
+  extern __shared__ __align__(16) uint8_t smem_raw[];
+  const TileSmem<KeyT, THREADS, IPT> s(smem_raw);
+
+  const int tid = threadIdx.x, lane = tid & 31, warp = tid >> 5;
+
+#ifdef TEZGPU_TICKET_ATOMIC
+  if (tid == 0) s.misc[0] = atomicAdd(tile_counter, 1u);
+#else
+  if (tid == 0) s.misc[0] = blockIdx.x;
+#endif
+  for (int i = tid; i < NWARPS * RADIX; i += THREADS) s.wcnt[i] = 0;
+#if TEZGPU_RANK_MODE == 2
+  for (int i = tid; i < NWARPS * RADIX; i += THREADS) s.wmask[i] = 0;
+#endif
+  if constexpr (IN == IO_RUNS)
+    for (int i = tid; i < TILE / 32; i += THREADS) s.dstart[i] = 0;
+  __syncthreads();
+  const uint32_t tile = s.misc[0];
+  const uint32_t tile_base = tile * (uint32_t)TILE;
+  const uint32_t tile_n = min((uint32_t)TILE, n - tile_base);
+  const uint32_t warp_base = (uint32_t)warp * 32u * IPT;
+
+  KeyT key[IPT];
+  uint32_t val[IPT];
+  if constexpr (IN == IO_RUNS) {
+    static_assert(TILE / 32 <= RADIX, "run-start bits fit s.dstart");
+    uint2 p[IPT];
+    load_run_items<THREADS, IPT>(reinterpret_cast<const uint2 *>(keys_in), runs, tile, tile_base, tile_n, s.pair, s.dstart, p);
+#pragma unroll
+    for (int j = 0; j < IPT; j++) {
+      key[j] = p[j].x;
+      val[j] = p[j].y;
+    }
+  } else {
+#pragma unroll
+    for (int j = 0; j < IPT; j++) {
+      const uint32_t li = warp_base + j * 32 + lane;
+      const bool valid = li < tile_n;
+      if constexpr (IN == IO_PAIR) {
+        uint2 p = make_uint2(~0u, 0u);
+        if (valid) p = reinterpret_cast<const uint2 *>(keys_in)[tile_base + li];
+        key[j] = p.x;
+        val[j] = p.y;
+      } else {
+        key[j] = valid ? keys_in[tile_base + li] : ~(KeyT)0;
+        val[j] = valid ? vals_in[tile_base + li] : 0u;
+      }
+    }
+  }
+  const uint32_t count = tile_rank_reorder<KeyT, THREADS, IPT>(
+      s, key, shift, [&](int j) { return val[j]; },
+      [&](uint32_t c) {
+        st_relaxed_gpu_u32(&tile_state[(size_t)tile * RADIX + tid], (tile == 0 ? STATE_FLAG_INCL : STATE_FLAG_LOCAL) | c);
+      });
 
   if (tid < RADIX) {
     uint32_t excl = 0;
@@ -244,7 +331,7 @@
       }
       st_relaxed_gpu_u32(&tile_state[(size_t)tile * RADIX + tid], STATE_FLAG_INCL | (excl + count));
     }
-    s_goff[tid] = hist_base[tid] + excl - s_dstart[tid];
+    s.goff[tid] = hist_base[tid] + excl - s.dstart[tid];
   }
   __syncthreads();
 
@@ -255,20 +342,96 @@
       KeyT kk;
       uint32_t v;
       if constexpr (PAIRS) {
-        const uint2 p = s_pair[slot];
+        const uint2 p = s.pair[slot];
         kk = p.x;
         v = p.y;
       } else {
-        kk = s_keys[slot];
-        v = s_vals[slot];
+        kk = s.keys[slot];
+        v = s.vals[slot];
       }
-      const uint32_t dest = s_goff[radix_digit(kk, shift)] + slot;
+      const uint32_t dest = s.goff[radix_digit(kk, shift)] + slot;
       if constexpr (OUT == IO_PAIR) {
         reinterpret_cast<uint2 *>(keys_out)[dest] = make_uint2((uint32_t)kk, v);
       } else {
         keys_out[dest] = kk;
         vals_out[dest] = v;
       }
+    }
+  }
+}
+
+template <int THREADS, int IPT>
+__global__ void __launch_bounds__(THREADS) k_runs_copy(const uint2 *__restrict__ blk, RadixRuns runs, uint32_t n,
+                                                       uint32_t *__restrict__ keys_out, uint32_t *__restrict__ vals_out) {
+  extern __shared__ __align__(16) uint8_t smem_raw[];
+  uint2 *s_runs = reinterpret_cast<uint2 *>(smem_raw);
+  uint32_t *s_bits = reinterpret_cast<uint32_t *>(s_runs + THREADS * IPT);
+  for (int i = threadIdx.x; i < IPT * THREADS / 32; i += THREADS) s_bits[i] = 0;
+  __syncthreads();
+  const uint32_t tile = blockIdx.x, tile_base = tile * (uint32_t)(THREADS * IPT);
+  const uint32_t tile_n = min((uint32_t)(THREADS * IPT), n - tile_base);
+  uint2 item[IPT];
+  load_run_items<THREADS, IPT>(blk, runs, tile, tile_base, tile_n, s_runs, s_bits, item);
+  const uint32_t pos0 = tile_base + (threadIdx.x >> 5) * 32u * IPT + (threadIdx.x & 31u);
+#pragma unroll
+  for (int j = 0; j < IPT; j++) {
+    const uint32_t pos = pos0 + j * 32u;
+    if (pos - tile_base < tile_n) {
+      keys_out[pos] = item[j].x;
+      vals_out[pos] = item[j].y;
+    }
+  }
+}
+
+
+__global__ void __launch_bounds__(1024) k_runs_count(const uint32_t *__restrict__ counts, uint32_t ntiles,
+                                                     uint32_t *__restrict__ nruns) {
+  __shared__ uint64_t s_warp[32];
+  const uint32_t *row = counts + (size_t)blockIdx.x * ntiles;
+  const uint32_t per = (ntiles + 1023) / 1024, t0 = threadIdx.x * per, t1 = min(t0 + per, ntiles);
+  uint64_t c = 0;
+  for (uint32_t t = t0; t < t1; t++) c += (row[t] & 0xFFFFu) != 0;
+  uint64_t total;
+  block_exclusive_scan_u64<1024>(c, s_warp, &total);
+  if (threadIdx.x == 0) nruns[blockIdx.x] = (uint32_t)total;
+}
+
+constexpr int RUNS_BUILD_IPT = 4;
+__global__ void __launch_bounds__(1024) k_runs_build(const uint32_t *__restrict__ counts, uint32_t ntiles, uint32_t stile,
+                                                     const uint32_t *__restrict__ hist_base, const uint32_t *__restrict__ nruns,
+                                                     uint32_t n, uint32_t ptile, uint32_t ptiles, uint2 *__restrict__ desc,
+                                                     uint32_t *__restrict__ first) {
+  __shared__ uint64_t s_warp[32];
+  __shared__ uint32_t s_k0;
+  const uint32_t d = blockIdx.x;
+  if (threadIdx.x == 0) s_k0 = 0;
+  __syncthreads();
+  if (threadIdx.x < d) atomicAdd(&s_k0, nruns[threadIdx.x]);
+  const uint32_t *row = counts + (size_t)d * ntiles;
+  uint64_t carry = 0;
+  for (uint32_t base = 0; base < ntiles; base += 1024 * RUNS_BUILD_IPT) {
+    const uint32_t t0 = base + threadIdx.x * RUNS_BUILD_IPT;
+    uint32_t w[RUNS_BUILD_IPT];
+    uint64_t v = 0;
+#pragma unroll
+    for (int i = 0; i < RUNS_BUILD_IPT; i++) {
+      w[i] = t0 + i < ntiles ? row[t0 + i] : 0u;
+      const uint32_t c = w[i] & 0xFFFFu;
+      v += c | ((uint64_t)(c != 0) << 32);
+    }
+    uint64_t total;
+    const uint64_t ex = carry + block_exclusive_scan_u64<1024>(v, s_warp, &total);
+    carry += total;
+    uint32_t pos = hist_base[d] + (uint32_t)ex, k = s_k0 + (uint32_t)(ex >> 32);
+#pragma unroll
+    for (int i = 0; i < RUNS_BUILD_IPT; i++) {
+      const uint32_t c = w[i] & 0xFFFFu;
+      if (!c) continue;
+      desc[k] = make_uint2(pos, (t0 + i) * stile + (w[i] >> 16));
+      for (uint32_t p = (pos + ptile - 1) / ptile; p < ptiles && p * ptile < pos + c; p++) first[p] = k;
+      pos += c;
+      if (pos == n) first[ptiles] = k;
+      k++;
     }
   }
 }
@@ -301,7 +464,7 @@
 template <typename KeyT, int IN, int OUT>
 static void radix_launch_pass(cudaStream_t st, uint32_t ntiles, const KeyT *kin, KeyT *kout, const uint32_t *vin,
                               uint32_t *vout, uint32_t n, int shift, const uint32_t *hist, uint32_t *state,
-                              uint32_t *counter) {
+                              uint32_t *counter, const RadixRuns &runs = RadixRuns()) {
   using T = RadixTuning<KeyT>;
   using Cfg = OnesweepCfg<KeyT, T::THREADS, T::IPT>;
   auto kern = k_onesweep_pass<KeyT, T::THREADS, T::IPT, T::MINB, IN, OUT>;
@@ -310,7 +473,7 @@
     TG_CUDA(cudaFuncSetAttribute(kern, cudaFuncAttributeMaxDynamicSharedMemorySize, (int)Cfg::SMEM));
     attr_set = true;
   }
-  kern<<<ntiles, T::THREADS, Cfg::SMEM, st>>>(kin, kout, vin, vout, n, shift, hist, state, counter);
+  kern<<<ntiles, T::THREADS, Cfg::SMEM, st>>>(kin, kout, vin, vout, n, shift, hist, state, counter, runs);
   TG_CUDA(cudaGetLastError());
 }
 
@@ -323,32 +486,64 @@
   return ntiles;
 }
 
-
-static int radix_sort_pairs(cudaStream_t st, const RadixWorkspace &ws, uint32_t *blk_a, uint32_t *blk_b, uint32_t n,
-                            int begin_bit, int npass, uint32_t pass_mask, int *launches) {
-  const int total = __builtin_popcount(pass_mask & ((1u << npass) - 1));
-  TG_CHECK(total >= 1, -1, "radix sort without a pass");
+static RadixRuns radix_build_runs(cudaStream_t st, const uint32_t *counts, uint32_t stage_tiles, uint32_t stage_tile,
+                                  const uint32_t *hist_base, uint32_t n, uint32_t *nruns_scratch, uint2 *desc,
+                                  uint32_t *first, int *launches) {
+  using T = RadixTuning<uint32_t>;
+  k_runs_count<<<RADIX, 1024, 0, st>>>(counts, stage_tiles, nruns_scratch);
+  k_runs_build<<<RADIX, 1024, 0, st>>>(counts, stage_tiles, stage_tile, hist_base, nruns_scratch, n, T::THREADS * T::IPT,
+                                       radix_num_tiles<uint32_t>(n), desc, first);
+  TG_CUDA(cudaGetLastError());
+  if (launches) *launches += 2;
+  RadixRuns r;
+  r.desc = desc;
+  r.first = first;
+  return r;
+}
+
+
+static uint32_t *radix_sort_pairs(cudaStream_t st, const RadixWorkspace &ws, const RadixRuns &runs, uint32_t *blk_a,
+                                  uint32_t *blk_b, uint32_t n, int begin_bit, int npass, uint32_t pass_mask, int *launches) {
+  using T = RadixTuning<uint32_t>;
+  const uint32_t mask = pass_mask & ((1u << npass) - 1);
+  TG_CHECK(mask != 0, -1, "radix sort without a pass");
+  const uint32_t rest = mask & (mask - 1);
   const uint32_t ntiles = radix_prepare<uint32_t>(st, ws, n, npass);
+  if (!rest) {
+    constexpr size_t smem = (size_t)T::THREADS * T::IPT * 8 + T::THREADS * T::IPT / 32 * 4;
+    static bool attr_set = false;
+    if (!attr_set) {
+      TG_CUDA(cudaFuncSetAttribute(k_runs_copy<T::THREADS, T::IPT>, cudaFuncAttributeMaxDynamicSharedMemorySize, (int)smem));
+      attr_set = true;
+    }
+    k_runs_copy<T::THREADS, T::IPT><<<ntiles, T::THREADS, smem, st>>>(reinterpret_cast<const uint2 *>(blk_b), runs, n, blk_a,
+                                                                      blk_a + n);
+    TG_CUDA(cudaGetLastError());
+    if (launches) (*launches)++;
+    return blk_a;
+  }
+  const int total = __builtin_popcount(rest);
+  uint32_t *in = blk_b, *out = blk_a;
   int done = 0;
   for (int p = 0; p < npass; p++) {
-    if (!((pass_mask >> p) & 1u)) continue;
-    uint32_t *in = (done & 1) ? blk_b : blk_a, *out = (done & 1) ? blk_a : blk_b;
+    if (!((rest >> p) & 1u)) continue;
     const bool first = done == 0, last = done + 1 == total;
     const int shift = begin_bit + p * RADIX_BITS;
     const uint32_t *hist = ws.hist + p * RADIX;
     uint32_t *state = ws.tile_state + (size_t)p * ntiles * RADIX, *counter = ws.tile_counter + p;
     if (first && last)
-      radix_launch_pass<uint32_t, IO_SEP_IOTA, IO_SEP>(st, ntiles, in, out, nullptr, out + n, n, shift, hist, state, counter);
+      radix_launch_pass<uint32_t, IO_RUNS, IO_SEP>(st, ntiles, in, out, nullptr, out + n, n, shift, hist, state, counter, runs);
     else if (first)
-      radix_launch_pass<uint32_t, IO_SEP_IOTA, IO_PAIR>(st, ntiles, in, out, nullptr, nullptr, n, shift, hist, state, counter);
+      radix_launch_pass<uint32_t, IO_RUNS, IO_PAIR>(st, ntiles, in, out, nullptr, nullptr, n, shift, hist, state, counter, runs);
     else if (last)
       radix_launch_pass<uint32_t, IO_PAIR, IO_SEP>(st, ntiles, in, out, nullptr, out + n, n, shift, hist, state, counter);
     else
       radix_launch_pass<uint32_t, IO_PAIR, IO_PAIR>(st, ntiles, in, out, nullptr, nullptr, n, shift, hist, state, counter);
     if (launches) (*launches)++;
     done++;
-  }
-  return done;
+    std::swap(in, out);
+  }
+  return in;
 }
 
 template <typename KeyT>
diff --git a/tez_b200/csrc/scan.cuh b/tez_b200/csrc/scan.cuh
--- a/tez_b200/csrc/scan.cuh
+++ b/tez_b200/csrc/scan.cuh
@@ -7,8 +7,8 @@
 constexpr int SCAN_IPT = 8;
 constexpr int SCAN_TILE = SCAN_THREADS * SCAN_IPT;
 
-__device__ __forceinline__ uint64_t block_exclusive_scan_u64(uint64_t v, uint64_t *s_warp ,
-                                                             uint64_t *total) {
+template <int NT = SCAN_THREADS>
+__device__ __forceinline__ uint64_t block_exclusive_scan_u64(uint64_t v, uint64_t *s_warp , uint64_t *total) {
   const int lane = threadIdx.x & 31, warp = threadIdx.x >> 5;
   uint64_t incl = v;
 #pragma unroll
@@ -20,7 +20,7 @@
   __syncthreads();
   uint64_t base = 0, tot = 0;
 #pragma unroll
-  for (int w = 0; w < SCAN_THREADS / 32; w++) {
+  for (int w = 0; w < NT / 32; w++) {
     uint64_t x = s_warp[w];
     if (w < warp) base += x;
     tot += x;
diff --git a/tez_b200/csrc/sorter.cuh b/tez_b200/csrc/sorter.cuh
--- a/tez_b200/csrc/sorter.cuh
+++ b/tez_b200/csrc/sorter.cuh
@@ -87,6 +87,17 @@
   return {FixedEmitKernel::PipeUnaligned, best};
 }
 
+template <bool FAST16>
+static int stage_ctas_per_sm() {
+  static int per_sm = 0;
+  if (!per_sm) {
+    TG_CUDA(cudaFuncSetAttribute(k_stage<FAST16>, cudaFuncAttributeMaxDynamicSharedMemorySize, (int)STAGE_SMEM));
+    TG_CUDA(cudaOccupancyMaxActiveBlocksPerMultiprocessor(&per_sm, k_stage<FAST16>, STAGE_THREADS, STAGE_SMEM));
+    per_sm = std::max(per_sm, 1);
+  }
+  return per_sm;
+}
+
 class SortPipeline {
  public:
   tezgpu_conf conf;
@@ -95,7 +106,7 @@
   EventTimer timer;
   int num_sms = 132;
 
-  DeviceBuffer sortA, sortB, same, blk, small, tile_state, sizes, rec_off;
+  DeviceBuffer sortA, sortB, same, blk, small, tile_state, sizes, rec_off, run_cnt, run_desc, run_first;
   DeviceBuffer t_pos[2], t_gid[2], t_lidx[2], t_key64[2], t_val[2], t_state, t_ghead, t_gneq, sym_sets, sym_tab, rep_flags;
   DeviceBuffer seg_start, tile_start, part_start, d_index, seg_crc, tile_desc, tile_crc, tie_state;
   PinnedBuffer h_small;
@@ -141,6 +152,7 @@
   uint32_t *d_m() { return small.as<uint32_t>() + 2072; }
   unsigned long long *d_ties() { return reinterpret_cast<unsigned long long *>(small.as<uint32_t>() + 2074); }
   uint32_t *d_ticket() { return small.as<uint32_t>() + 2073; }
+  uint32_t *d_nruns() { return small.as<uint32_t>() + 3072; }
   unsigned long long *d_dups() { return reinterpret_cast<unsigned long long *>(small.as<uint32_t>() + 2066); }
   uint64_t *d_totals() { return reinterpret_cast<uint64_t *>(small.as<uint32_t>() + 2068); }
 
@@ -289,18 +301,33 @@
       delete t;
     }
     if (n) {
+      uint32_t pass_mask = 0xF;
+      if (unordered) {
+        pass_mask = 0;
+        for (int q = 0; q < 4; q++) if (8 * q + 8 > 32 - pbits) pass_mask |= 1u << q;
+        if (!pass_mask) pass_mask = 1;
+      }
+      const int stage_shift = RADIX_BITS * __builtin_ctz(pass_mask);
+      const uint32_t stiles = (uint32_t)div_up(n, STAGE_TILE);
+      run_cnt.ensure((size_t)RADIX * stiles * 4);
+      run_desc.ensure(std::min<size_t>(n, (size_t)RADIX * stiles) * 8);
+      run_first.ensure(((size_t)radix_num_tiles<uint32_t>(n) + 1) * 4);
       TG_CUDA(cudaMemsetAsync(same.p, 0, n, stream));
       const bool fast16 = rec.fixed && !rec.key_off && !rec.use_runs && rec.klen == 16 && ((rec.klen + rec.vlen) % 16 == 0) && rec.cmp == CMP_BYTES &&
                           (((uintptr_t)rec.kv & 15u) == 0);
-      int sgrid = (int)std::min<uint64_t>(div_up(n, 256), (uint64_t)num_sms * 16);
-      if (fast16) k_stage<true><<<sgrid, 256, 0, stream>>>(rec, K, d_hist(), d_error());
-      else k_stage<false><<<sgrid, 256, 0, stream>>>(rec, K, d_hist(), d_error());
+      const uint32_t sgrid = (uint32_t)std::min<uint64_t>(stiles, (uint64_t)num_sms * (fast16 ? stage_ctas_per_sm<true>() : stage_ctas_per_sm<false>()));
+      if (fast16)
+        k_stage<true><<<sgrid, STAGE_THREADS, STAGE_SMEM, stream>>>(rec, stage_shift, sortB.as<uint2>(), run_cnt.as<uint32_t>(), stiles, d_hist(), d_error());
+      else
+        k_stage<false><<<sgrid, STAGE_THREADS, STAGE_SMEM, stream>>>(rec, stage_shift, sortB.as<uint2>(), run_cnt.as<uint32_t>(), stiles, d_hist(), d_error());
       TG_CUDA(cudaGetLastError());
       k_radix_scan_hist<<<1, RADIX, 0, stream>>>(d_hist(), 4, n, d_trivial());
       TG_CUDA(cudaGetLastError());
       launches += 2;
       timer.mark(stream);
 
+      const RadixRuns runs = radix_build_runs(stream, run_cnt.as<uint32_t>(), stiles, STAGE_TILE, d_hist() + stage_shift / RADIX_BITS * RADIX,
+                                              n, d_nruns(), run_desc.as<uint2>(), run_first.as<uint32_t>(), &launches);
       RadixWorkspace ws;
       ws.hist = d_hist();
       ws.trivial = d_trivial();
@@ -308,14 +335,9 @@
       ws.tile_state_words = radix_tile_state_words<uint32_t>(n, 4);
       tile_state.ensure(ws.tile_state_words * 4);
       ws.tile_state = tile_state.as<uint32_t>();
-      uint32_t pass_mask = 0xF;
-      if (unordered) {
-        pass_mask = 0;
-        for (int q = 0; q < 4; q++) if (8 * q + 8 > 32 - pbits) pass_mask |= 1u << q;
-        if (!pass_mask) pass_mask = 1;
-      }
-      int done = radix_sort_pairs(stream, ws, sortA.as<uint32_t>(), sortB.as<uint32_t>(), n, 0, 4, pass_mask, &launches);
-      if (done & 1) { K = sortB.as<uint32_t>(); order = sortB.as<uint32_t>() + n; }
+      uint32_t *res = radix_sort_pairs(stream, ws, runs, sortA.as<uint32_t>(), sortB.as<uint32_t>(), n, 0, 4, pass_mask, &launches);
+      K = res;
+      order = res + n;
       if (unordered) {
         k_flip_order<<<(uint32_t)div_up(n, 256), 256, 0, stream>>>(order, n);
         launches++;
diff --git a/tez_b200/csrc/sorter_kernels.cuh b/tez_b200/csrc/sorter_kernels.cuh
--- a/tez_b200/csrc/sorter_kernels.cuh
+++ b/tez_b200/csrc/sorter_kernels.cuh
@@ -141,61 +141,137 @@
   return compose_sort_word(r, p, prefix, bad);
 }
 
+__device__ __forceinline__ uint32_t stage_record_word(const Records &r, uint32_t i, bool &bad, int *__restrict__ error_flag) {
+  uint64_t koff;
+  uint32_t klen, vlen;
+  int32_t run_part = 0;
+  if (r.fixed && r.use_runs) {
+    const unsigned am = __activemask();
+    const int leader = __ffs(am) - 1;
+    uint32_t seg = (int)(threadIdx.x & 31) == leader ? run_of(r.runs, i) : 0u;
+    seg = __shfl_sync(am, seg, leader);
+    while (seg + 1 < r.runs.nseg && i >= __ldg(r.runs.rec_base + seg + 1)) seg++;
+    const uint64_t roff = __ldg(r.runs.seg_off + seg) + (uint64_t)(i - __ldg(r.runs.rec_base + seg)) * r.runs.rec_size;
+    koff = roff + r.runs.hdr_len;
+    klen = r.klen;
+    vlen = r.vlen;
+    run_part = (int32_t)__ldg(r.runs.seg_part + seg);
+    bool ok = true;
+    for (uint32_t b = 0; b < r.runs.hdr_len; b++) ok &= r.kv[roff + b] == (uint8_t)(r.runs.hdr_bytes >> (8 * b));
+    if (!ok) atomicOr(error_flag, 2);
+  } else {
+    record_lookup(r, i, koff, klen, vlen);
+  }
+  const int32_t given = r.hash_partition ? 0 : ((r.fixed && r.use_runs) ? run_part : (r.partition ? r.partition[i] : 0));
+  return stage_sort_word(r, r.kv + koff, klen, given, bad);
+}
+
+#ifndef TEZGPU_STAGE_IPT
+#define TEZGPU_STAGE_IPT 16
+#endif
+#ifndef TEZGPU_STAGE_BATCH
+#define TEZGPU_STAGE_BATCH 8
+#endif
+constexpr int STAGE_THREADS = 384;
+constexpr int STAGE_IPT = TEZGPU_STAGE_IPT;
+constexpr uint32_t STAGE_TILE = (uint32_t)STAGE_THREADS * STAGE_IPT;
+constexpr int STAGE_LOAD_BATCH = TEZGPU_STAGE_BATCH;
+using StageCfg = OnesweepCfg<uint32_t, STAGE_THREADS, STAGE_IPT>;
+constexpr size_t STAGE_SMEM = StageCfg::SMEM + 4 * RADIX * 4;
+static_assert(STAGE_TILE < 65536, "tile-local digit starts and counts are packed into 16 bits");
+
 template <bool FAST16>
-__global__ void __launch_bounds__(256) k_stage(Records r, uint32_t *__restrict__ keys_out, uint32_t *__restrict__ hist,
-                                               int *__restrict__ error_flag) {
-  __shared__ uint32_t s_hist[4 * RADIX];
-  for (int i = threadIdx.x; i < 4 * RADIX; i += blockDim.x) s_hist[i] = 0;
+__global__ void __launch_bounds__(STAGE_THREADS, 2) k_stage(Records r, int shift, uint2 *__restrict__ blk,
+                                                            uint32_t *__restrict__ counts, uint32_t ntiles,
+                                                            uint32_t *__restrict__ hist, int *__restrict__ error_flag) {
+  constexpr int IPT = STAGE_IPT;
+  extern __shared__ __align__(16) uint8_t smem_raw[];
+  const TileSmem<uint32_t, STAGE_THREADS, IPT> s(smem_raw);
+  uint32_t *s_hist = reinterpret_cast<uint32_t *>(smem_raw + StageCfg::SMEM);
+  const int tid = threadIdx.x, lane = tid & 31, warp = tid >> 5;
+  const int q0 = shift / RADIX_BITS;
+  for (int i = tid; i < 4 * RADIX; i += STAGE_THREADS) s_hist[i] = 0;
+  for (int i = tid; i < StageCfg::NWARPS * RADIX; i += STAGE_THREADS) s.wmask[i] = 0;
+  const uint32_t n = r.n;
+  const uint32_t warp_base = (uint32_t)warp * 32u * IPT;
+  for (uint32_t tile = blockIdx.x; tile < ntiles; tile += gridDim.x) {
+    for (int i = tid; i < StageCfg::NWARPS * RADIX; i += STAGE_THREADS) s.wcnt[i] = 0;
+    __syncthreads();
+    const uint32_t tile_base = tile * STAGE_TILE;
+    const uint32_t tile_n = min(STAGE_TILE, n - tile_base);
+    uint32_t key[IPT];
+    bool bad = false;
+    if constexpr (FAST16) {
+      const uint64_t stride = r.klen + r.vlen;
+#pragma unroll
+      for (int j0 = 0; j0 < IPT; j0 += STAGE_LOAD_BATCH) {
+        uint4 kq[STAGE_LOAD_BATCH];
+        int32_t gp[STAGE_LOAD_BATCH];
+#pragma unroll
+        for (int b = 0; b < STAGE_LOAD_BATCH && j0 + b < IPT; b++) {
+          const uint32_t li = warp_base + (j0 + b) * 32 + lane;
+          kq[b] = make_uint4(0, 0, 0, 0);
+          gp[b] = 0;
+          if (li < tile_n) {
+            const uint32_t i = r.unordered ? n - 1u - (tile_base + li) : tile_base + li;
+            kq[b] = *reinterpret_cast<const uint4 *>(r.kv + (uint64_t)i * stride);
+            if (!r.hash_partition && r.partition) gp[b] = r.partition[i];
+          }
+        }
+#pragma unroll
+        for (int b = 0; b < STAGE_LOAD_BATCH && j0 + b < IPT; b++) {
+          const uint32_t li = warp_base + (j0 + b) * 32 + lane;
+          int32_t p = gp[b];
+          if (r.hash_partition) {
+            uint32_t h = 1;
+            const uint32_t w[4] = {kq[b].x, kq[b].y, kq[b].z, kq[b].w};
+#pragma unroll
+            for (int k = 0; k < 16; k++) h = 31u * h + (uint32_t)(int32_t)(int8_t)((w[k >> 2] >> (8 * (k & 3))) & 0xFF);
+            p = (int32_t)((h & 0x7fffffffu) % (uint32_t)r.num_partitions);
+          }
+          bool bb;
+          const uint32_t K = compose_sort_word(r, p, __byte_perm(kq[b].x, 0, 0x0123), bb);
+          key[j0 + b] = li < tile_n ? K : ~0u;
+          bad |= li < tile_n && bb;
+        }
+      }
+    } else {
+#pragma unroll 4
+      for (int j = 0; j < IPT; j++) {
+        const uint32_t li = warp_base + j * 32 + lane;
+        key[j] = ~0u;
+        if (li < tile_n) {
+          bool bb;
+          key[j] = stage_record_word(r, r.unordered ? n - 1u - (tile_base + li) : tile_base + li, bb, error_flag);
+          bad |= bb;
+        }
+      }
+    }
+    if (bad) atomicOr(error_flag, 1);
+#pragma unroll
+    for (int j = 0; j < IPT; j++) {
+      if (warp_base + j * 32 + lane < tile_n) {
+#pragma unroll
+        for (int q = 0; q < 4; q++)
+          if (q != q0) atomicAdd(&s_hist[q * RADIX + ((key[j] >> (8 * q)) & 0xFF)], 1u);
+      }
+    }
+    uint32_t count = tile_rank_reorder<uint32_t, STAGE_THREADS, IPT>(
+        s, key, shift, [&](int j) { return tile_base + warp_base + j * 32 + lane; }, [](uint32_t) {});
+    __syncthreads();
+    if (tid < RADIX) {
+      if (tid == RADIX - 1) count -= STAGE_TILE - tile_n;
+      s_hist[q0 * RADIX + tid] += count;
+      counts[(size_t)tid * ntiles + tile] = (s.dstart[tid] << 16) | count;
+    }
+#pragma unroll
+    for (int k = 0; k < IPT; k++) {
+      const uint32_t slot = (uint32_t)tid + k * STAGE_THREADS;
+      if (slot < tile_n) blk[tile_base + slot] = s.pair[slot];
+    }
+  }
   __syncthreads();
-  const uint32_t stride = gridDim.x * blockDim.x;
-  for (uint32_t i = blockIdx.x * blockDim.x + threadIdx.x; i < r.n; i += stride) {
-    uint32_t K;
-    bool bad;
-    if (FAST16) {
-      const uint4 kq = *reinterpret_cast<const uint4 *>(r.kv + (uint64_t)i * (r.klen + r.vlen));
-      const uint32_t prefix = __byte_perm(kq.x, 0, 0x0123);
-      int32_t p;
-      if (r.hash_partition) {
-        uint32_t h = 1;
-        const uint32_t w[4] = {kq.x, kq.y, kq.z, kq.w};
-#pragma unroll
-        for (int k = 0; k < 16; k++) h = 31u * h + (uint32_t)(int32_t)(int8_t)((w[k >> 2] >> (8 * (k & 3))) & 0xFF);
-        p = (int32_t)((h & 0x7fffffffu) % (uint32_t)r.num_partitions);
-      } else {
-        p = r.partition ? r.partition[i] : 0;
-      }
-      K = compose_sort_word(r, p, prefix, bad);
-    } else {
-      uint64_t koff;
-      uint32_t klen, vlen;
-      int32_t run_part = 0;
-      if (r.fixed && r.use_runs) {
-        const unsigned am = __activemask();
-        const int leader = __ffs(am) - 1;
-        uint32_t seg = (int)(threadIdx.x & 31) == leader ? run_of(r.runs, i) : 0u;
-        seg = __shfl_sync(am, seg, leader);
-        while (seg + 1 < r.runs.nseg && i >= __ldg(r.runs.rec_base + seg + 1)) seg++;
-        const uint64_t roff = __ldg(r.runs.seg_off + seg) + (uint64_t)(i - __ldg(r.runs.rec_base + seg)) * r.runs.rec_size;
-        koff = roff + r.runs.hdr_len;
-        klen = r.klen;
-        vlen = r.vlen;
-        run_part = (int32_t)__ldg(r.runs.seg_part + seg);
-        bool ok = true;
-        for (uint32_t b = 0; b < r.runs.hdr_len; b++) ok &= r.kv[roff + b] == (uint8_t)(r.runs.hdr_bytes >> (8 * b));
-        if (!ok) atomicOr(error_flag, 2);
-      } else {
-        record_lookup(r, i, koff, klen, vlen);
-      }
-      const int32_t given = r.hash_partition ? 0 : ((r.fixed && r.use_runs) ? run_part : (r.partition ? r.partition[i] : 0));
-      K = stage_sort_word(r, r.kv + koff, klen, given, bad);
-    }
-    if (bad) atomicOr(error_flag, 1);
-    keys_out[r.unordered ? r.n - 1u - i : i] = K;
-#pragma unroll
-    for (int q = 0; q < 4; q++) atomicAdd(&s_hist[q * RADIX + ((K >> (8 * q)) & 0xFF)], 1u);
-  }
-  __syncthreads();
-  for (int i = threadIdx.x; i < 4 * RADIX; i += blockDim.x) {
+  for (int i = tid; i < 4 * RADIX; i += STAGE_THREADS) {
     uint32_t c = s_hist[i];
     if (c) atomicAdd(&hist[i], c);
   }
```
